# ComputationalRobotics/cuADMM

Hardware: NVIDIA B200
Metric: ADMM iterations/s (higher is better)
Workload: dtype f64

## Files before the change

### cuadmm_b200/csrc/chol_host.cpp

```cpp
#include "chol_host.h"
#include "common.h"
#include <algorithm>
#include <cmath>
#include <numeric>
#include <stdlib.h>

namespace cuadmm {

SymCsc form_aat(int64_t m, int64_t ncols, const int32_t* rowptr, const int32_t* colind, const double* val, double eps) {
    const int64_t nnz = rowptr[m];
    std::vector<int64_t> cp(ncols + 1, 0);
    for (int64_t p = 0; p < nnz; ++p) cp[colind[p] + 1]++;
    for (int64_t k = 0; k < ncols; ++k) cp[k + 1] += cp[k];
    std::vector<int32_t> ci(nnz);
    std::vector<double> cx(nnz);
    {
        std::vector<int64_t> nx(cp.begin(), cp.end() - 1);
        for (int64_t i = 0; i < m; ++i)
            for (int p = rowptr[i]; p < rowptr[i + 1]; ++p) {
                const int64_t q = nx[colind[p]]++;
                ci[q] = (int32_t)i;
                cx[q] = val[p];
            }
    }
    SymCsc M;
    M.n = m;
    M.p.assign(m + 1, 0);
    std::vector<double> acc(m, 0.0);
    std::vector<int32_t> mark(m, -1);
    std::vector<int32_t> list;
    for (int64_t i = 0; i < m; ++i) {
        list.clear();
        mark[i] = (int32_t)i;
        list.push_back((int32_t)i);
        acc[i] = eps;
        for (int p = rowptr[i]; p < rowptr[i + 1]; ++p) {
            const int64_t k = colind[p];
            const double aik = val[p];
            const int32_t* lo = std::lower_bound(ci.data() + cp[k], ci.data() + cp[k + 1], (int32_t)i);
            for (int64_t q = lo - ci.data(); q < cp[k + 1]; ++q) {
                const int32_t j = ci[q];
                if (mark[j] != (int32_t)i) { mark[j] = (int32_t)i; acc[j] = 0.0; list.push_back(j); }
                acc[j] += aik * cx[q];
            }
        }
        std::sort(list.begin(), list.end());
        for (int32_t j : list) { M.i.push_back(j); M.x.push_back(acc[j]); }
        M.p[i + 1] = (int64_t)M.i.size();
    }
    return M;
}

std::vector<int32_t> min_degree_order(const SymCsc& M) {
    const int64_t n = M.n;
    std::vector<int32_t> perm(n);
    if (n == 0) return perm;
    std::vector<std::vector<int32_t>> vadj(n), eadj(n), members(n);
    {
        std::vector<int32_t> cnt(n, 0);
        for (int64_t j = 0; j < n; ++j)
            for (int64_t p = M.p[j]; p < M.p[j + 1]; ++p) if (M.i[p] != j) { cnt[j]++; cnt[M.i[p]]++; }
        for (int64_t j = 0; j < n; ++j) vadj[j].reserve(cnt[j]);
        for (int64_t j = 0; j < n; ++j)
            for (int64_t p = M.p[j]; p < M.p[j + 1]; ++p) if (M.i[p] != j) { vadj[j].push_back(M.i[p]); vadj[M.i[p]].push_back((int32_t)j); }
    }
    enum { VAR = 0, ELEM = 1, DEAD = 2 };
    std::vector<uint8_t> status(n, VAR);
    std::vector<int64_t> degree(n);
    std::vector<int32_t> head(n + 1, -1), next(n, -1), prev(n, -1);
    auto list_insert = [&](int32_t i) {
        const int64_t d = degree[i];
        next[i] = head[d]; prev[i] = -1;
        if (head[d] >= 0) prev[head[d]] = i;
        head[d] = i;
    };
    auto list_remove = [&](int32_t i) {
        const int64_t d = degree[i];
        if (prev[i] >= 0) next[prev[i]] = next[i]; else head[d] = next[i];
        if (next[i] >= 0) prev[next[i]] = prev[i];
    };
    for (int64_t i = 0; i < n; ++i) { degree[i] = (int64_t)vadj[i].size(); }
    for (int64_t i = n - 1; i >= 0; --i) list_insert((int32_t)i);
    std::vector<int64_t> mark(n, -1), wstamp(n, -1), w(n, 0);
    std::vector<int32_t> Lp;
    int64_t mindeg = 0;
    std::vector<int64_t> blocked(n, -1);
    std::vector<int32_t> cands;
    int64_t k = 0, round = 0;
    auto eliminate = [&](const int32_t p) {
        list_remove(p);
        perm[k] = p;
        Lp.clear();
        mark[p] = k;
        for (int32_t v : vadj[p]) if (status[v] == VAR && mark[v] != k) { mark[v] = k; Lp.push_back(v); }
        for (int32_t e : eadj[p]) if (status[e] == ELEM) {
            for (int32_t v : members[e]) if (status[v] == VAR && mark[v] != k) { mark[v] = k; Lp.push_back(v); }
            status[e] = DEAD;
            std::vector<int32_t>().swap(members[e]);
        }
        status[p] = ELEM;
        std::vector<int32_t>().swap(vadj[p]);
        std::vector<int32_t>().swap(eadj[p]);
        const int64_t lp = (int64_t)Lp.size();
        for (int32_t i : Lp) {
            list_remove(i);
            auto& E = eadj[i];
            size_t o = 0;
            for (size_t t = 0; t < E.size(); ++t) {
                const int32_t e = E[t];
                if (status[e] != ELEM) continue;
                if (wstamp[e] != k) { wstamp[e] = k; w[e] = (int64_t)members[e].size(); }
                w[e] -= 1;
                E[o++] = e;
            }
            E.resize(o);
        }
        for (int32_t i : Lp) {
            auto& A = vadj[i];
            size_t o = 0;
            for (size_t t = 0; t < A.size(); ++t) {
                const int32_t v = A[t];
                if (status[v] == VAR && mark[v] != k) A[o++] = v;
            }
            A.resize(o);
            int64_t d = (int64_t)o + (lp - 1);
            auto& E = eadj[i];
            size_t oe = 0;
            for (size_t t = 0; t < E.size(); ++t) {
                const int32_t e = E[t];
                if (status[e] != ELEM) continue;
                if (w[e] <= 0) {
                    status[e] = DEAD;
                    std::vector<int32_t>().swap(members[e]);
                    continue;
                }
                d += w[e];
                E[oe++] = e;
            }
            E.resize(oe);
            E.push_back(p);
            d = std::min<int64_t>(d, n - k - 1);
            d = std::min<int64_t>(d, degree[i] + lp - 1);
            if (d < 0) d = 0;
            degree[i] = d;
        }
        members[p] = Lp;
        for (int32_t i : Lp) {
            list_insert(i);
            blocked[i] = round;
            if (degree[i] < mindeg) mindeg = degree[i];
        }
        ++k;
    };
    const char* slack_env = getenv("CUADMM_MD_SLACK");
    const int64_t slack_pct = slack_env ? atoll(slack_env) : 25;
    while (k < n) {
        ++round;
        while (head[mindeg] < 0) ++mindeg;
        const int64_t limit = std::min<int64_t>(n, mindeg + std::max<int64_t>(1, mindeg * slack_pct / 100));
        cands.clear();
        for (int64_t d = mindeg; d <= limit; ++d)
            for (int32_t i = head[d]; i >= 0; i = next[i]) cands.push_back(i);
        for (int32_t p : cands) {
            if (status[p] != VAR || blocked[p] == round || degree[p] > limit) continue;
            eliminate(p);
        }
    }
    return perm;
}

static SymCsc permute_lower(const SymCsc& M, const std::vector<int32_t>& perm, std::vector<int32_t>& iperm) {
    const int64_t n = M.n;
    iperm.assign(n, 0);
    for (int64_t k = 0; k < n; ++k) iperm[perm[k]] = (int32_t)k;
    SymCsc C;
    C.n = n;
    C.p.assign(n + 1, 0);
    const int64_t nnz = M.p[n];
    for (int64_t j = 0; j < n; ++j)
        for (int64_t p = M.p[j]; p < M.p[j + 1]; ++p) {
            const int32_t a = iperm[j], b = iperm[M.i[p]];
            C.p[std::min(a, b) + 1]++;
        }
    for (int64_t j = 0; j < n; ++j) C.p[j + 1] += C.p[j];
    C.i.resize(nnz); C.x.resize(nnz);
    std::vector<int64_t> nx(C.p.begin(), C.p.end() - 1);
    for (int64_t j = 0; j < n; ++j)
        for (int64_t p = M.p[j]; p < M.p[j + 1]; ++p) {
            const int32_t a = iperm[j], b = iperm[M.i[p]];
            const int64_t q = nx[std::min(a, b)]++;
            C.i[q] = std::max(a, b);
            C.x[q] = M.x[p];
        }
    std::vector<std::pair<int32_t, double>> tmp;
    for (int64_t j = 0; j < n; ++j) {
        tmp.clear();
        for (int64_t p = C.p[j]; p < C.p[j + 1]; ++p) tmp.emplace_back(C.i[p], C.x[p]);
        std::sort(tmp.begin(), tmp.end(), [](const std::pair<int32_t, double>& a, const std::pair<int32_t, double>& b) { return a.first < b.first; });
        for (size_t t = 0; t < tmp.size(); ++t) { C.i[C.p[j] + t] = tmp[t].first; C.x[C.p[j] + t] = tmp[t].second; }
    }
    return C;
}

static void lower_rows(const SymCsc& C, std::vector<int64_t>& rp, std::vector<int32_t>& rj, std::vector<double>& rx) {
    const int64_t n = C.n;
    rp.assign(n + 1, 0);
    for (int64_t j = 0; j < n; ++j)
        for (int64_t p = C.p[j]; p < C.p[j + 1]; ++p) rp[C.i[p] + 1]++;
    for (int64_t i = 0; i < n; ++i) rp[i + 1] += rp[i];
    rj.resize(rp[n]); rx.resize(rp[n]);
    std::vector<int64_t> nx(rp.begin(), rp.end() - 1);
    for (int64_t j = 0; j < n; ++j)
        for (int64_t p = C.p[j]; p < C.p[j + 1]; ++p) {
            const int64_t q = nx[C.i[p]]++;
            rj[q] = (int32_t)j;
            rx[q] = C.x[p];
        }
}

void chol_symbolic(const SymCsc& M, const std::vector<int32_t>& perm, CholFactor& F, SymCsc* permuted) {
    const int64_t n = M.n;
    F.n = n;
    F.perm = perm;
    SymCsc C = permute_lower(M, perm, F.iperm);
    std::vector<int64_t> rp; std::vector<int32_t> rj; std::vector<double> rx;
    lower_rows(C, rp, rj, rx);
    F.parent.assign(n, -1);
    std::vector<int32_t> ancestor(n, -1);
    for (int64_t k = 0; k < n; ++k) {
        for (int64_t p = rp[k]; p < rp[k + 1]; ++p) {
            int32_t i = rj[p];
            while (i != -1 && i < k) {
                const int32_t inext = ancestor[i];
                ancestor[i] = (int32_t)k;
                if (inext == -1) F.parent[i] = (int32_t)k;
                i = inext;
            }
        }
    }
    std::vector<int64_t> cnt(n, 1);
    std::vector<int32_t> flag(n, -1);
    for (int pass = 0; pass < 2; ++pass) {
        std::vector<int64_t> nx;
        if (pass == 1) {
            F.Lp.assign(n + 1, 0);
            for (int64_t j = 0; j < n; ++j) F.Lp[j + 1] = F.Lp[j] + cnt[j];
            F.Li.assign(F.Lp[n], 0);
            F.Lx.assign(F.Lp[n], 0.0);
            nx.assign(F.Lp.begin(), F.Lp.end() - 1);
            for (int64_t j = 0; j < n; ++j) F.Li[nx[j]++] = (int32_t)j;
            std::fill(flag.begin(), flag.end(), -1);
        }
        for (int64_t k = 0; k < n; ++k) {
            flag[k] = (int32_t)k;
            for (int64_t p = rp[k]; p < rp[k + 1]; ++p) {
                int32_t i = rj[p];
                while (i != -1 && i < k && flag[i] != (int32_t)k) {
                    flag[i] = (int32_t)k;
                    if (pass == 0) cnt[i]++; else F.Li[nx[i]++] = (int32_t)k;
                    i = F.parent[i];
                }
            }
        }
    }
    if (permuted) *permuted = std::move(C);
}

std::vector<int32_t> postorder_perm(const SymCsc& M, const std::vector<int32_t>& perm) {
    CholFactor F;
    chol_symbolic(M, perm, F, nullptr);
    const int64_t n = F.n;
    std::vector<int32_t> head(n, -1), nxt(n, -1);
    for (int64_t j = n - 1; j >= 0; --j) if (F.parent[j] >= 0) { nxt[j] = head[F.parent[j]]; head[F.parent[j]] = (int32_t)j; }
    std::vector<int32_t> post; post.reserve(n);
    std::vector<int32_t> stack;
    for (int64_t r = 0; r < n; ++r) {
        if (F.parent[r] >= 0) continue;
        stack.push_back((int32_t)r);
        while (!stack.empty()) {
            const int32_t v = stack.back();
            const int32_t c = head[v];
            if (c >= 0) { head[v] = nxt[c]; stack.push_back(c); }
            else { post.push_back(v); stack.pop_back(); }
        }
    }
    std::vector<int32_t> out(n);
    for (int64_t k = 0; k < n; ++k) out[k] = perm[post[k]];
    return out;
}

std::vector<int64_t> find_supernodes(const CholFactor& F, int64_t max_size) {
    const int64_t n = F.n;
    std::vector<int64_t> sn;
    sn.push_back(0);
    std::vector<int32_t> nchild(n, 0);
    for (int64_t j = 0; j < n; ++j) if (F.parent[j] >= 0) nchild[F.parent[j]]++;
    for (int64_t j = 1; j < n; ++j) {
        const int64_t cprev = F.Lp[j] - F.Lp[j - 1], ccur = F.Lp[j + 1] - F.Lp[j];
        const bool join = F.parent[j - 1] == j && ccur == cprev - 1 && nchild[j] == 1 && (j - sn.back()) < max_size;
        if (!join) sn.push_back(j);
    }
    if (n > 0) sn.push_back(n);
    return sn;
}

double pivot_tol() {
    if (const char* e = getenv("CUADMM_PIVOT_TOL")) { const double v = atof(e); if (v > 0.0 && v < 1.0) return v; }
    return 1e-11;
}

void chol_numeric(const SymCsc& C, CholFactor& F, int64_t n_lead) {
    F.n_deficient = 0;
    const double kPivotTol = pivot_tol();
    const int64_t n = F.n;
    std::vector<int64_t> rp; std::vector<int32_t> rj; std::vector<double> rx;
    lower_rows(C, rp, rj, rx);
    std::vector<double> x(n, 0.0);
    std::vector<int64_t> c(n);
    for (int64_t j = 0; j < n; ++j) c[j] = F.Lp[j] + 1;
    std::vector<int32_t> flag(n, -1), stack(n), path(n);
    for (int64_t k = 0; k < n; ++k) {
        int64_t top = n;
        flag[k] = (int32_t)k;
        double d = 0.0, mkk = 0.0;
        for (int64_t p = rp[k]; p < rp[k + 1]; ++p) {
            int32_t i = rj[p];
            if (i == k) { d = rx[p]; mkk = rx[p]; continue; }
            x[i] = rx[p];
            int64_t len = 0;
            while (i != -1 && i < k && flag[i] != (int32_t)k) {
                path[len++] = i;
                flag[i] = (int32_t)k;
                i = F.parent[i];
            }
            while (len > 0) stack[--top] = path[--len];
        }
        for (; top < n; ++top) {
            const int32_t i = stack[top];
            if (i >= n_lead) { x[i] = 0.0; continue; }
            const double lki = x[i] / F.Lx[F.Lp[i]];
            x[i] = 0.0;
            const int64_t pend = c[i];
            if (k < n_lead) {
                for (int64_t p = F.Lp[i] + 1; p < pend; ++p) x[F.Li[p]] -= F.Lx[p] * lki;
            } else {
                for (int64_t p = F.Lp[i] + 1; p < pend && F.Li[p] < n_lead; ++p) x[F.Li[p]] -= F.Lx[p] * lki;
            }
            d -= lki * lki;
            F.Lx[pend] = lki;
            c[i] = pend + 1;
        }
        if (k < n_lead) {
            if (!(d > kPivotTol * std::max(mkk, 1e-300))) {
                F.Lx[F.Lp[k]] = INFINITY;
                F.n_deficient++;
            } else {
                F.Lx[F.Lp[k]] = std::sqrt(d);
            }
        } else {
            F.Lx[F.Lp[k]] = d;
        }
    }
}

}
```

### cuadmm_b200/csrc/chol_host.h

```cpp
#pragma once
#include <stdint.h>
#include <vector>

namespace cuadmm {

struct SymCsc {
    int64_t n = 0;
    std::vector<int64_t> p;
    std::vector<int32_t> i;
    std::vector<double> x;
};

SymCsc form_aat(int64_t m, int64_t ncols, const int32_t* rowptr, const int32_t* colind, const double* val, double eps);

std::vector<int32_t> min_degree_order(const SymCsc& M);

struct CholFactor {
    int64_t n = 0;
    std::vector<int32_t> perm, iperm;
    std::vector<int32_t> parent;
    std::vector<int64_t> Lp;
    std::vector<int32_t> Li;
    std::vector<double> Lx;
    int64_t n_deficient = 0;
    int64_t nnz() const { return Lp.empty() ? 0 : Lp[n]; }
};

std::vector<int32_t> postorder_perm(const SymCsc& M, const std::vector<int32_t>& perm);

std::vector<int64_t> find_supernodes(const CholFactor& F, int64_t max_size);

void chol_symbolic(const SymCsc& M, const std::vector<int32_t>& perm, CholFactor& F, SymCsc* permuted = nullptr);
double pivot_tol();
void chol_numeric(const SymCsc& Mperm, CholFactor& F, int64_t n_lead);

}
```

### cuadmm_b200/csrc/debug_api.cpp

```cpp
#include "chol_host.h"
#include "common.h"
#include <algorithm>
#include <cmath>

using namespace cuadmm;

extern "C" {

int cuadmm_debug_chol_solve(int64_t m, int64_t ncols, const int32_t* rowptr, const int32_t* colind, const double* val,
                            double eps, double n_lead_frac, const double* rhs, double* y, int32_t* perm_out,
                            int64_t* stats ) {
    return guarded([&] {
        SymCsc M = form_aat(m, ncols, rowptr, colind, val, eps);
        std::vector<int32_t> perm = min_degree_order(M);
        perm = postorder_perm(M, perm);
        CholFactor F; SymCsc C;
        chol_symbolic(M, perm, F, &C);
        const int64_t n_lead = std::max<int64_t>(0, std::min<int64_t>(m, (int64_t)(n_lead_frac * (double)m)));
        chol_numeric(C, F, n_lead);
        const int64_t r = m - n_lead;
        std::vector<double> S((size_t)(r * r), 0.0);
        for (int64_t j = n_lead; j < m; ++j)
            for (int64_t p = C.p[j]; p < C.p[j + 1]; ++p) S[(C.i[p] - n_lead) + (j - n_lead) * r] = C.x[p];
        for (int64_t j = 0; j < n_lead; ++j)
            for (int64_t p = F.Lp[j] + 1; p < F.Lp[j + 1]; ++p) if (F.Li[p] >= n_lead)
                for (int64_t q = p; q < F.Lp[j + 1]; ++q)
                    S[(F.Li[q] - n_lead) + (F.Li[p] - n_lead) * r] -= F.Lx[q] * F.Lx[p];
        for (int64_t k = 0; k < r; ++k) {
            double d = S[k + k * r];
            d = (d > 1e-11) ? std::sqrt(d) : INFINITY; S[k + k * r] = d;
            for (int64_t i = k + 1; i < r; ++i) S[i + k * r] /= d;
            for (int64_t j = k + 1; j < r; ++j)
                for (int64_t i = j; i < r; ++i) S[i + j * r] -= S[i + k * r] * S[j + k * r];
        }
        std::vector<double> z(m);
        for (int64_t k = 0; k < m; ++k) z[k] = rhs[F.perm[k]];
        for (int64_t j = 0; j < n_lead; ++j) {
            z[j] /= F.Lx[F.Lp[j]];
            for (int64_t p = F.Lp[j] + 1; p < F.Lp[j + 1]; ++p) z[F.Li[p]] -= F.Lx[p] * z[j];
        }
        for (int64_t j = 0; j < r; ++j) {
            z[n_lead + j] /= S[j + j * r];
            for (int64_t i = j + 1; i < r; ++i) z[n_lead + i] -= S[i + j * r] * z[n_lead + j];
        }
        for (int64_t j = r - 1; j >= 0; --j) {
            for (int64_t i = j + 1; i < r; ++i) z[n_lead + j] -= S[i + j * r] * z[n_lead + i];
            z[n_lead + j] /= S[j + j * r];
        }
        for (int64_t j = n_lead - 1; j >= 0; --j) {
            for (int64_t p = F.Lp[j] + 1; p < F.Lp[j + 1]; ++p) z[j] -= F.Lx[p] * z[F.Li[p]];
            z[j] /= F.Lx[F.Lp[j]];
        }
        for (int64_t k = 0; k < m; ++k) y[F.perm[k]] = z[k];
        if (perm_out) std::copy(F.perm.begin(), F.perm.end(), perm_out);
        if (stats) {
            stats[0] = M.p[m]; stats[1] = F.nnz(); stats[2] = F.n_deficient;
            std::vector<int32_t> lev(m, 0);
            int32_t depth = 0;
            for (int64_t j = 0; j < m; ++j) {
                for (int64_t p = F.Lp[j] + 1; p < F.Lp[j + 1]; ++p) lev[F.Li[p]] = std::max(lev[F.Li[p]], lev[j] + 1);
                depth = std::max(depth, lev[j] + 1);
            }
            stats[3] = depth;
            std::vector<int64_t> cnt(depth + 1, 0);
            for (int64_t j = 0; j < m; ++j) cnt[lev[j]]++;
            int64_t narrow = 0;
            for (int32_t l = 0; l < depth; ++l) if (cnt[l] < 8) narrow += cnt[l];
            stats[4] = narrow;
            std::vector<int64_t> sn = find_supernodes(F, 256);
            const int64_t nsn = (int64_t)sn.size() - 1;
            std::vector<int32_t> snof(m, 0), slev(std::max<int64_t>(nsn, 1), 0);
            for (int64_t s = 0; s < nsn; ++s) for (int64_t j = sn[s]; j < sn[s + 1]; ++j) snof[j] = (int32_t)s;
            int32_t sdepth = 0;
            for (int64_t s = 0; s < nsn; ++s) {
                for (int64_t j = sn[s]; j < sn[s + 1]; ++j)
                    for (int64_t p = F.Lp[j] + 1; p < F.Lp[j + 1]; ++p) {
                        const int32_t t = snof[F.Li[p]];
                        if (t != s) slev[t] = std::max(slev[t], slev[s] + 1);
                    }
                sdepth = std::max(sdepth, slev[s] + 1);
            }
            stats[5] = nsn; stats[6] = sdepth;
            std::vector<int64_t> scnt(sdepth + 1, 0);
            for (int64_t s = 0; s < nsn; ++s) scnt[slev[s]] += sn[s + 1] - sn[s];
            int64_t deep_rows = 0;
            for (int32_t l = 48; l < sdepth; ++l) deep_rows += scnt[l];
            stats[7] = deep_rows;
        }
    });
}

}
```

### cuadmm_b200/csrc/dense.cu

```cuda
#include "dense.h"
#include <stdio.h>
#include <stdlib.h>
#include <algorithm>

namespace cuadmm {

static constexpr int GB_M = 64, GB_N = 64, GB_K = 16, GB_PAD = 4;

__device__ __forceinline__ void dmma_m8n8k4(double& c0, double& c1, double a, double b) {
    asm volatile("mma.sync.aligned.m8n8k4.row.col.f64.f64.f64.f64 {%0,%1}, {%2}, {%3}, {%0,%1};"
                 : "+d"(c0), "+d"(c1) : "d"(a), "d"(b));
}

template <bool TA, bool TB>
__global__ void __launch_bounds__(128) dgemm_kernel(int64_t m, int64_t n, int64_t k, double alpha,
                                                    const double* __restrict__ A, int64_t lda,
                                                    const double* __restrict__ B, int64_t ldb,
                                                    double beta, double* C, int64_t ldc, int shape) {
    if (shape == 1 && (int64_t)blockIdx.y * GB_N > (int64_t)blockIdx.x * GB_M + (GB_M - 1)) return;
    __shared__ double As[2][GB_K][GB_M + GB_PAD];
    __shared__ double Bs[2][GB_K][GB_N + GB_PAD];
    const int tid = threadIdx.x, lane = tid & 31, warp = tid >> 5;
    const int wm = (warp & 1) * 32, wn = (warp >> 1) * 32;
    const int64_t m0 = (int64_t)blockIdx.x * GB_M, n0 = (int64_t)blockIdx.y * GB_N;
    double acc[4][4][2];
#pragma unroll
    for (int i = 0; i < 4; ++i)
#pragma unroll
        for (int j = 0; j < 4; ++j) { acc[i][j][0] = 0.0; acc[i][j][1] = 0.0; }

    auto load_tiles = [&](int buf, int64_t k0) {
#pragma unroll
        for (int t = 0; t < 8; ++t) {
            const int e = tid + t * 128;
            int mm, kk;
            if (TA) { kk = e % GB_K; mm = e / GB_K; } else { mm = e % GB_M; kk = e / GB_M; }
            const int64_t gm = m0 + mm, gk = k0 + kk;
            double v = 0.0;
            if (gm < m && gk < k) v = TA ? A[gk + gm * lda] : A[gm + gk * lda];
            As[buf][kk][mm] = v;
        }
#pragma unroll
        for (int t = 0; t < 8; ++t) {
            const int e = tid + t * 128;
            int nn, kk;
            if (TB) { nn = e % GB_N; kk = e / GB_N; } else { kk = e % GB_K; nn = e / GB_K; }
            const int64_t gn = n0 + nn, gk = k0 + kk;
            double v = 0.0;
            if (gn < n && gk < k) v = TB ? B[gn + gk * ldb] : B[gk + gn * ldb];
            Bs[buf][kk][nn] = v;
        }
    };

    const int64_t nk = (k + GB_K - 1) / GB_K;
    const int64_t kt0 = (shape == 2) ? ((n0 / GB_K < nk) ? n0 / GB_K : nk) : 0;
    if (nk > kt0) load_tiles((int)(kt0 & 1), kt0 * GB_K);
    __syncthreads();
    for (int64_t kt = kt0; kt < nk; ++kt) {
        const int buf = (int)(kt & 1);
        if (kt + 1 < nk) load_tiles(buf ^ 1, (kt + 1) * GB_K);
#pragma unroll
        for (int kk = 0; kk < GB_K; kk += 4) {
            double a[4], b[4];
#pragma unroll
            for (int i = 0; i < 4; ++i) a[i] = As[buf][kk + (lane & 3)][wm + i * 8 + (lane >> 2)];
#pragma unroll
            for (int j = 0; j < 4; ++j) b[j] = Bs[buf][kk + (lane & 3)][wn + j * 8 + (lane >> 2)];
#pragma unroll
            for (int i = 0; i < 4; ++i)
#pragma unroll
                for (int j = 0; j < 4; ++j) dmma_m8n8k4(acc[i][j][0], acc[i][j][1], a[i], b[j]);
        }
        __syncthreads();
    }
#pragma unroll
    for (int i = 0; i < 4; ++i)
#pragma unroll
        for (int j = 0; j < 4; ++j)
#pragma unroll
            for (int h = 0; h < 2; ++h) {
                const int64_t gm = m0 + wm + i * 8 + (lane >> 2);
                const int64_t gn = n0 + wn + j * 8 + (lane & 3) * 2 + h;
                if (gm < m && gn < n) {
                    double* c = C + gm + gn * ldc;
                    *c = (beta == 0.0) ? alpha * acc[i][j][h] : alpha * acc[i][j][h] + beta * (*c);
                }
            }
}

void dgemm(cudaStream_t st, bool transA, bool transB, int64_t m, int64_t n, int64_t k, double alpha,
           const double* A, int64_t lda, const double* B, int64_t ldb, double beta, double* C, int64_t ldc, int shape) {
    if (m <= 0 || n <= 0) return;
    dim3 grid((unsigned)((m + GB_M - 1) / GB_M), (unsigned)((n + GB_N - 1) / GB_N));
    if (!transA && !transB) dgemm_kernel<false, false><<<grid, 128, 0, st>>>(m, n, k, alpha, A, lda, B, ldb, beta, C, ldc, shape);
    else if (!transA && transB) dgemm_kernel<false, true><<<grid, 128, 0, st>>>(m, n, k, alpha, A, lda, B, ldb, beta, C, ldc, shape);
    else if (transA && !transB) dgemm_kernel<true, false><<<grid, 128, 0, st>>>(m, n, k, alpha, A, lda, B, ldb, beta, C, ldc, shape);
    else dgemm_kernel<true, true><<<grid, 128, 0, st>>>(m, n, k, alpha, A, lda, B, ldb, beta, C, ldc, shape);
    CUADMM_CUDA(cudaGetLastError());
}

static constexpr int NB = 64;

__global__ void __launch_bounds__(256) potf2_inv_kernel(int nb, double* A, int64_t lda, double* inv, int* info, int blk_index, const double* pivot_floor) {
    extern __shared__ double potf2_smem[];
    double (*S)[NB + 1] = reinterpret_cast<double (*)[NB + 1]>(potf2_smem);
    double (*I)[NB + 1] = reinterpret_cast<double (*)[NB + 1]>(potf2_smem + NB * (NB + 1));
    __shared__ int bad;
    const int tid = threadIdx.x;
    if (tid == 0) bad = 0;
    for (int e = tid; e < nb * nb; e += 256) { const int i = e % nb, j = e / nb; S[i][j] = (i >= j) ? A[i + j * lda] : 0.0; }
    __syncthreads();
    for (int kk = 0; kk < nb; ++kk) {
        if (tid == 0) {
            const double d = S[kk][kk];
            const double fl = pivot_floor ? pivot_floor[kk] : 0.0;
            if (!(d > fl)) { bad = 1; S[kk][kk] = INFINITY; } else S[kk][kk] = sqrt(d);
        }
        __syncthreads();
        const double dk = S[kk][kk];
        for (int i = kk + 1 + tid; i < nb; i += 256) S[i][kk] /= dk;
        __syncthreads();
        const int rem = nb - kk - 1;
        for (int e = tid; e < rem * rem; e += 256) {
            const int i = kk + 1 + e % rem, j = kk + 1 + e / rem;
            if (i >= j) S[i][j] -= S[i][kk] * S[j][kk];
        }
        __syncthreads();
    }
    if (tid < nb) {
        const int j = tid;
        for (int i = 0; i < nb; ++i) {
            double s = (i == j) ? 1.0 : 0.0;
            for (int t = j; t < i; ++t) s -= S[i][t] * I[t][j];
            I[i][j] = (i >= j) ? s / S[i][i] : 0.0;
        }
    }
    __syncthreads();
    for (int e = tid; e < nb * nb; e += 256) {
        const int i = e % nb, j = e / nb;
        if (i >= j) A[i + j * lda] = S[i][j];
        if (inv) inv[i + (int64_t)j * NB] = I[i][j];
    }
    if (tid == 0 && bad && info) atomicAdd(info, 1);
}

void potrf_lower(cudaStream_t st, int64_t n, double* A, int64_t lda, double* inv_diag, int* d_info, const double* pivot_floor) {
    DevBuf<double> tmp(std::max<int64_t>(n * NB, 1));
    DevBuf<double> inv_local;
    if (!inv_diag) { inv_local.alloc(std::max<int64_t>(n * NB, 1)); inv_diag = inv_local.p; }
    const size_t potf2_bytes = sizeof(double) * 2 * NB * (NB + 1);
    CUADMM_CUDA(cudaFuncSetAttribute((const void*)potf2_inv_kernel, cudaFuncAttributeMaxDynamicSharedMemorySize, (int)potf2_bytes));
    for (int64_t j = 0; j < n; j += NB) {
        const int nb = (int)std::min<int64_t>(NB, n - j);
        double* Ajj = A + j + j * lda;
        double* invj = inv_diag + j * NB;
        potf2_inv_kernel<<<1, 256, potf2_bytes, st>>>(nb, Ajj, lda, invj, d_info, (int)(j / NB), pivot_floor ? pivot_floor + j : nullptr);
        const int64_t below = n - j - nb;
        if (below > 0) {
            double* Aij = A + (j + nb) + j * lda;
            dgemm(st, false, true, below, nb, nb, 1.0, Aij, lda, invj, NB, 0.0, tmp.p, below);
            CUADMM_CUDA(cudaMemcpy2DAsync(Aij, sizeof(double) * lda, tmp.p, sizeof(double) * below,
                                          sizeof(double) * below, nb, cudaMemcpyDeviceToDevice, st));
            double* A22 = A + (j + nb) + (j + nb) * lda;
            dgemm(st, false, true, below, below, nb, -1.0, Aij, lda, Aij, lda, 1.0, A22, lda, 1);
        }
    }
    CUADMM_CUDA(cudaGetLastError());
    CUADMM_CUDA(cudaStreamSynchronize(st));
}

__global__ void copy_inv_block_kernel(int nb, const double* __restrict__ inv, double* X, int64_t ldx) {
    for (int e = threadIdx.x; e < nb * nb; e += blockDim.x) {
        const int i = e % nb, j = e / nb;
        X[i + j * ldx] = inv[i + (int64_t)j * NB];
    }
}

void trtri_lower(cudaStream_t st, int64_t n, const double* L, int64_t ldl, const double* inv_diag, double* X, int64_t ldx) {
    CUADMM_CUDA(cudaMemset2DAsync(X, sizeof(double) * ldx, 0, sizeof(double) * n, n, st));
    DevBuf<double> T(std::max<int64_t>((int64_t)NB * n, 1));
    for (int64_t i = 0; i < n; i += NB) {
        const int nb = (int)std::min<int64_t>(NB, n - i);
        const double* invi = inv_diag + i * NB;
        copy_inv_block_kernel<<<1, 256, 0, st>>>(nb, invi, X + i + i * ldx, ldx);
        if (i > 0) {
            dgemm(st, false, false, nb, i, i, 1.0, L + i, ldl, X, ldx, 0.0, T.p, NB, 2);
            dgemm(st, false, false, nb, i, nb, -1.0, invi, NB, T.p, NB, 0.0, X + i, ldx);
        }
    }
    CUADMM_CUDA(cudaGetLastError());
    CUADMM_CUDA(cudaStreamSynchronize(st));
}

__global__ void scatter_coo_kernel(int64_t nnz, const int32_t* __restrict__ r, const int32_t* __restrict__ c,
                                   const double* __restrict__ v, double* D, int64_t ld, int symmetric) {
    const int64_t e = (int64_t)blockIdx.x * blockDim.x + threadIdx.x;
    if (e >= nnz) return;
    D[r[e] + (int64_t)c[e] * ld] = v[e];
    if (symmetric && r[e] != c[e]) D[c[e] + (int64_t)r[e] * ld] = v[e];
}

__global__ void transpose_kernel(int64_t n, const double* __restrict__ in, double* __restrict__ out) {
    __shared__ double tile[32][33];
    const int64_t bx = (int64_t)blockIdx.x * 32, by = (int64_t)blockIdx.y * 32;
    for (int j = threadIdx.y; j < 32; j += blockDim.y) {
        const int64_t x = bx + threadIdx.x, y = by + j;
        if (x < n && y < n) tile[j][threadIdx.x] = in[x + y * n];
    }
    __syncthreads();
    for (int j = threadIdx.y; j < 32; j += blockDim.y) {
        const int64_t x = by + threadIdx.x, y = bx + j;
        if (x < n && y < n) out[x + y * n] = tile[threadIdx.x][j];
    }
}

__global__ void tile_occupancy_kernel(int64_t r, int nt, const double* __restrict__ A, int* __restrict__ flags) {
    const int I = blockIdx.y, J = blockIdx.x;
    int any = 0;
    for (int e = threadIdx.x; e < 64 * 64; e += blockDim.x) {
        const int64_t i = (int64_t)I * 64 + e / 64, j = (int64_t)J * 64 + e % 64;
        if (i < r && j < r && A[i * r + j] != 0.0) any = 1;
    }
    if (__syncthreads_or(any) && threadIdx.x == 0) flags[I * nt + J] = 1;
}

void build_dense_tail(const SymCsc& C, const CholFactor& F, int64_t n_lead, int64_t r,
                      DevBuf<double>& tail_inv, DevBuf<double>& tail_inv_t, int64_t* n_deficient,
                      std::vector<int>* tile_flags) {
    cudaStream_t st = 0;
    DevBuf<double> S(r * r);
    S.zero(st);
    {
        std::vector<int32_t> rr, cc; std::vector<double> vv;
        for (int64_t j = n_lead; j < n_lead + r; ++j)
            for (int64_t p = C.p[j]; p < C.p[j + 1]; ++p) { rr.push_back((int32_t)(C.i[p] - n_lead)); cc.push_back((int32_t)(j - n_lead)); vv.push_back(C.x[p]); }
        if (!vv.empty()) {
            DevBuf<int32_t> dr, dc; DevBuf<double> dv;
            dr.upload(rr, st); dc.upload(cc, st); dv.upload(vv, st);
            scatter_coo_kernel<<<(unsigned)((vv.size() + 255) / 256), 256, 0, st>>>((int64_t)vv.size(), dr.p, dc.p, dv.p, S.p, r, 1);
            CUADMM_CUDA(cudaStreamSynchronize(st));
        }
    }
    {
        std::vector<int64_t> cols;
        for (int64_t j = 0; j < n_lead; ++j)
            if (F.Lp[j + 1] > F.Lp[j] + 1 && F.Li[F.Lp[j + 1] - 1] >= n_lead) cols.push_back(j);
        const int64_t budget = (int64_t)1 << 27;
        const int64_t cw = std::max<int64_t>(64, std::min<int64_t>((int64_t)cols.size(), budget / std::max<int64_t>(r, 1)));
        DevBuf<double> B(r * std::min<int64_t>(cw, std::max<int64_t>((int64_t)cols.size(), 1)));
        std::vector<int32_t> rr, cc; std::vector<double> vv;
        for (int64_t c0 = 0; c0 < (int64_t)cols.size(); c0 += cw) {
            const int64_t w = std::min<int64_t>(cw, (int64_t)cols.size() - c0);
            rr.clear(); cc.clear(); vv.clear();
            for (int64_t t = 0; t < w; ++t) {
                const int64_t j = cols[c0 + t];
                for (int64_t p = F.Lp[j + 1] - 1; p > F.Lp[j] && F.Li[p] >= n_lead; --p) {
                    rr.push_back((int32_t)(F.Li[p] - n_lead)); cc.push_back((int32_t)t); vv.push_back(F.Lx[p]);
                }
            }
            CUADMM_CUDA(cudaMemsetAsync(B.p, 0, sizeof(double) * (size_t)(r * w), st));
            DevBuf<int32_t> dr, dc; DevBuf<double> dv;
            dr.upload(rr, st); dc.upload(cc, st); dv.upload(vv, st);
            scatter_coo_kernel<<<(unsigned)((vv.size() + 255) / 256), 256, 0, st>>>((int64_t)vv.size(), dr.p, dc.p, dv.p, B.p, r, 0);
            dgemm(st, false, true, r, r, w, -1.0, B.p, r, B.p, r, 1.0, S.p, r, 1);
            CUADMM_CUDA(cudaStreamSynchronize(st));
        }
    }
    DevBuf<double> inv_diag(std::max<int64_t>(r * NB, 1));
    DevBuf<int> info(1);
    info.zero(st);
    std::vector<double> h_floor(r, 0.0);
    for (int64_t j = n_lead; j < n_lead + r; ++j)
        for (int64_t p = C.p[j]; p < C.p[j + 1]; ++p) if (C.i[p] == j) h_floor[j - n_lead] = pivot_tol() * C.x[p];
    DevBuf<double> d_floor; d_floor.upload(h_floor, st);
    potrf_lower(st, r, S.p, r, inv_diag.p, info.p, d_floor.p);
    int h_info = 0;
    info.download(&h_info, 1, st);
    CUADMM_CUDA(cudaStreamSynchronize(st));
    if (n_deficient) *n_deficient = h_info;
    tail_inv_t.alloc(r * r);
    trtri_lower(st, r, S.p, r, inv_diag.p, tail_inv_t.p, r);
    tail_inv.alloc(r * r);
    dim3 grid((unsigned)((r + 31) / 32), (unsigned)((r + 31) / 32)), block(32, 8);
    transpose_kernel<<<grid, block, 0, st>>>(r, tail_inv_t.p, tail_inv.p);
    CUADMM_CUDA(cudaGetLastError());
    CUADMM_CUDA(cudaStreamSynchronize(st));
    {
        const int nt = (int)((r + 63) / 64);
        DevBuf<int> flags((int64_t)nt * nt);
        flags.zero(st);
        tile_occupancy_kernel<<<dim3(nt, nt), 256, 0, st>>>(r, nt, tail_inv.p, flags.p);
        std::vector<int> h((size_t)nt * nt);
        flags.download(h.data(), (int64_t)h.size(), st);
        CUADMM_CUDA(cudaStreamSynchronize(st));
        if (getenv("CUADMM_YSOLVE_VERBOSE")) {
            int64_t lower = 0, used = 0;
            for (int I = 0; I < nt; ++I) for (int J = 0; J <= I; ++J) { ++lower; used += h[(size_t)I * nt + J]; }
            fprintf(stderr, "[ysolve] dense tail %lld: %lld of %lld lower 64x64 tiles of L22^-1 are non-zero (%.1f%%)\n",
                    (long long)r, (long long)used, (long long)lower, 100.0 * (double)used / (double)lower);
        }
        if (tile_flags) tile_flags->swap(h);
    }
}

}
```

### cuadmm_b200/csrc/dense.h

```cpp
#pragma once
#include "common.h"
#include "chol_host.h"

namespace cuadmm {

void dgemm(cudaStream_t st, bool transA, bool transB, int64_t m, int64_t n, int64_t k, double alpha,
           const double* A, int64_t lda, const double* B, int64_t ldb, double beta, double* C, int64_t ldc, int shape = 0);

void potrf_lower(cudaStream_t st, int64_t n, double* A, int64_t lda, double* inv_diag, int* d_info,
                 const double* pivot_floor = nullptr);
void trtri_lower(cudaStream_t st, int64_t n, const double* L, int64_t ldl, const double* inv_diag, double* Linv, int64_t ldi);

void build_dense_tail(const SymCsc& Cperm, const CholFactor& F, int64_t n_lead, int64_t n_tail,
                      DevBuf<double>& tail_inv, DevBuf<double>& tail_inv_t, int64_t* n_deficient = nullptr,
                      std::vector<int>* tile_flags = nullptr);

}
```

### cuadmm_b200/csrc/ysolve.cu

```cuda
#include "ysolve.h"
#include <chrono>
#include <thread>
#include <atomic>
#include "dense.h"
#include <algorithm>
#include <numeric>
#include <stdio.h>
#include <stdlib.h>

namespace cuadmm {

static constexpr int kTriThreads = 256;
static constexpr int kLongRowNnz = 24;
static constexpr int kNarrowSlots = 160;
static constexpr int kNarrowThreads = 1024;

struct SlotWork {
    static constexpr int K = 4;
    int32_t u; int is_long;
    double rv, invd;
    int64_t p, p1; int step;
    int32_t d[K]; double v[K];

    __device__ __forceinline__ void load(int64_t s, int lane, const int32_t* __restrict__ slot_rows,
            const int32_t* __restrict__ slot_info, const int64_t* __restrict__ ptr, const int32_t* __restrict__ dep,
            const double* __restrict__ val, const double* __restrict__ inv_diag, const double* __restrict__ rhs,
            const int32_t* __restrict__ rhs_gather) {
        is_long = slot_info[s] >> 30;
        u = slot_rows[8 * s + (is_long ? 0 : (lane >> 2))];
        step = is_long ? 32 : 4;
        p = 0; p1 = 0; rv = 0.0; invd = 0.0;
        if (u >= 0) {
            p = ptr[u] + (is_long ? lane : (lane & 3));
            p1 = ptr[u + 1];
            invd = inv_diag[u];
            rv = rhs_gather ? rhs[rhs_gather[u]] : rhs[u];
        }
#pragma unroll
        for (int k = 0; k < K; ++k) {
            const int64_t q = p + (int64_t)k * step;
            if (q < p1) { d[k] = dep[q]; v[k] = val[q]; } else { d[k] = -1; v[k] = 0.0; }
        }
    }
    __device__ __forceinline__ void finish(int lane, const int32_t* __restrict__ dep, const double* __restrict__ val,
                                           double* x, double* out_scatter, const int32_t* __restrict__ out_perm) {
        double acc = 0.0;
#pragma unroll
        for (int k = 0; k < K; ++k) if (d[k] >= 0) acc = fma(v[k], x[d[k]], acc);
        for (int64_t q = p + (int64_t)K * step; q < p1; q += step) acc = fma(val[q], x[dep[q]], acc);
        acc += __shfl_xor_sync(0xffffffffu, acc, 1);
        acc += __shfl_xor_sync(0xffffffffu, acc, 2);
        if (is_long) {
            acc += __shfl_xor_sync(0xffffffffu, acc, 4);
            acc += __shfl_xor_sync(0xffffffffu, acc, 8);
            acc += __shfl_xor_sync(0xffffffffu, acc, 16);
        }
        const bool writer = (u >= 0) && (is_long ? (lane == 0) : ((lane & 3) == 0));
        if (writer) {
            const double r = (rv - acc) * invd;
            x[u] = r;
            if (out_scatter) out_scatter[out_perm[u]] = r;
        }
    }
};

#define CUADMM_TRI_PARAMS                                                                                   \
    const int32_t* __restrict__ slot_rows, const int32_t* __restrict__ slot_info, const int64_t* __restrict__ ptr, \
    const int32_t* __restrict__ dep, const double* __restrict__ val, const double* __restrict__ inv_diag,   \
    const double* __restrict__ rhs, const int32_t* __restrict__ rhs_gather, double* x, double* out_scatter, \
    const int32_t* __restrict__ out_perm, const int* __restrict__ done_flag
#define CUADMM_TRI_LOAD(W, S) (W).load((S), lane, slot_rows, slot_info, ptr, dep, val, inv_diag, rhs, rhs_gather)
#define CUADMM_TRI_FINISH(W) (W).finish(lane, dep, val, x, out_scatter, out_perm)

__global__ void __launch_bounds__(kTriThreads) tri_wide_kernel(int64_t slot0, int64_t slot1, CUADMM_TRI_PARAMS) {
    if (done_flag && *done_flag) return;
    const int lane = threadIdx.x & 31;
    const int64_t s = slot0 + (((int64_t)blockIdx.x * kTriThreads + threadIdx.x) >> 5);
    if (s >= slot1) return;
    SlotWork w;
    CUADMM_TRI_LOAD(w, s);
    CUADMM_TRI_FINISH(w);
}

template <int NW>
__device__ __forceinline__ void tri_level_loop(const int64_t* __restrict__ lvl_ptr, int level0, int level1, int lane, int warp,
        CUADMM_TRI_PARAMS) {
    (void)done_flag;
    if (level0 >= level1) return;
    SlotWork w;
    int64_t s0 = lvl_ptr[level0];
    int64_t s1 = lvl_ptr[level0 + 1];
    bool have = (s0 + warp) < s1;
    if (have) CUADMM_TRI_LOAD(w, s0 + warp);
    for (int l = level0; l < level1; ++l) {
        if (have) {
            CUADMM_TRI_FINISH(w);
            for (int64_t s = s0 + warp + NW; s < s1; s += NW) { SlotWork t; CUADMM_TRI_LOAD(t, s); CUADMM_TRI_FINISH(t); }
        }
        s0 = s1;
        have = false;
        if (l + 1 < level1) {
            s1 = lvl_ptr[l + 2];
            have = (s0 + warp) < s1;
            if (have) CUADMM_TRI_LOAD(w, s0 + warp);
        }
        __syncthreads();
    }
}

__global__ void __launch_bounds__(kNarrowThreads) tri_narrow_kernel(int level0, int level1, const int64_t* __restrict__ level_ptr,
                                                                    CUADMM_TRI_PARAMS) {
    if (done_flag && *done_flag) return;
    tri_level_loop<kNarrowThreads / 32>(level_ptr, level0, level1, threadIdx.x & 31, threadIdx.x >> 5,
        slot_rows, slot_info, ptr, dep, val, inv_diag, rhs, rhs_gather, x, out_scatter, out_perm, done_flag);
}

__global__ void __launch_bounds__(kTriThreads) tri_subtree_kernel(const int64_t* __restrict__ sub_off,
        const int64_t* __restrict__ sub_lvl_ptr, CUADMM_TRI_PARAMS) {
    if (done_flag && *done_flag) return;
    const int64_t base = sub_off[blockIdx.x];
    const int nl = (int)(sub_off[blockIdx.x + 1] - base) - 1;
    tri_level_loop<kTriThreads / 32>(sub_lvl_ptr + base, 0, nl, threadIdx.x & 31, threadIdx.x >> 5,
        slot_rows, slot_info, ptr, dep, val, inv_diag, rhs, rhs_gather, x, out_scatter, out_perm, done_flag);
}

#ifndef CUADMM_PK_CHUNK
#define CUADMM_PK_CHUNK 65536
#endif
#ifndef CUADMM_PK_RING
#define CUADMM_PK_RING 2
#endif
static constexpr int kPkChunk = CUADMM_PK_CHUNK;
static constexpr int kPkRing = CUADMM_PK_RING;
#ifndef CUADMM_PK_THREADS
#define CUADMM_PK_THREADS 1024
#endif
static constexpr int kPkThreads = CUADMM_PK_THREADS;
static constexpr int kPkRecHeader = 8 + 32 + 16 + 16 + 16 + 64;
static constexpr int kPkMaxRowEntries = 768;
static constexpr int kPkMaxRows = 23000;
static constexpr int kPkChainMax = 384;

__device__ __forceinline__ uint32_t smem_u32(const void* p) { return (uint32_t)__cvta_generic_to_shared(p); }

__device__ __forceinline__ long long pk_globaltimer() {
    long long t;
    asm volatile("mov.u64 %0, %%globaltimer;" : "=l"(t));
    return t;
}

__device__ __forceinline__ void pk_fetch(unsigned char* dst, const unsigned char* src, uint64_t* bar) {
    asm volatile("mbarrier.arrive.expect_tx.shared::cta.b64 _, [%0], %1;" :: "r"(smem_u32(bar)), "r"(kPkChunk) : "memory");
    asm volatile("cp.async.bulk.shared::cluster.global.mbarrier::complete_tx::bytes [%0], [%1], %2, [%3];"
                 :: "r"(smem_u32(dst)), "l"(src), "r"(kPkChunk), "r"(smem_u32(bar)) : "memory");
}

__device__ __forceinline__ void pk_wait(uint64_t* bar, uint32_t parity) {
    uint32_t ok;
    do {
        asm volatile("{ .reg .pred p; mbarrier.try_wait.parity.shared::cta.b64 p, [%1], %2; selp.u32 %0, 1, 0, p; }"
                     : "=r"(ok) : "r"(smem_u32(bar)), "r"(parity) : "memory");
    } while (!ok);
}

__device__ __forceinline__ void pk_record(const unsigned char* rec, int lane, double* xs) {
    const int r = lane >> 2;
    const bool is_long = *reinterpret_cast<const int32_t*>(rec) != 0;
    const int ul = reinterpret_cast<const int32_t*>(rec + 8)[r];
    const int voff = reinterpret_cast<const uint16_t*>(rec + 40)[r];
    const int ioff = reinterpret_cast<const uint16_t*>(rec + 56)[r];
    const int ln = reinterpret_cast<const uint16_t*>(rec + 72)[r];
    const double invd = reinterpret_cast<const double*>(rec + 88)[r];
    const int j = is_long ? lane : (lane & 3);
    const int step = is_long ? 32 : 4;
    const double* val = reinterpret_cast<const double*>(rec) + voff;
    const uint16_t* idx = reinterpret_cast<const uint16_t*>(rec) + ioff;
    const double cur = ul >= 0 ? xs[ul] : 0.0;
    double acc = 0.0;
    for (int k = j; k < ln; k += step) acc = fma(val[k], xs[idx[k]], acc);
    acc += __shfl_xor_sync(0xffffffffu, acc, 1);
    acc += __shfl_xor_sync(0xffffffffu, acc, 2);
    if (is_long) {
        acc += __shfl_xor_sync(0xffffffffu, acc, 4);
        acc += __shfl_xor_sync(0xffffffffu, acc, 8);
        acc += __shfl_xor_sync(0xffffffffu, acc, 16);
    }
    if (ul >= 0 && j == 0) xs[ul] = (cur - acc) * invd;
}

static constexpr int kPkHeavyExt = 8;

__global__ void __launch_bounds__(256) pk_gather_kernel(int64_t n_rows, int main_blocks, const int32_t* __restrict__ heavy,
        int n_heavy, const int32_t* __restrict__ prow_src, const int64_t* __restrict__ ext_ptr,
        const int32_t* __restrict__ ext_dep, const double* __restrict__ ext_val, const double* __restrict__ rhs,
        const double* __restrict__ x, double* __restrict__ w, const int* __restrict__ done_flag) {
    if (done_flag && *done_flag) return;
    if ((int)blockIdx.x < main_blocks) {
        const int64_t g = (int64_t)blockIdx.x * 256 + threadIdx.x;
        if (g >= n_rows) return;
        const int32_t src = prow_src[g];
        double acc = src >= 0 ? rhs[src] : 0.0;
        if (ext_ptr) {
            const int64_t p0 = ext_ptr[g], p1 = ext_ptr[g + 1];
            if (p1 - p0 > kPkHeavyExt) return;
            for (int64_t p = p0; p < p1; ++p) acc = fma(-ext_val[p], x[ext_dep[p]], acc);
        }
        w[g] = acc;
    } else {
        const int lane = threadIdx.x & 31;
        const int hw = ((int)blockIdx.x - main_blocks) * 8 + (threadIdx.x >> 5);
        if (hw >= n_heavy) return;
        const int64_t g = heavy[hw];
        double acc = 0.0;
        for (int64_t p = ext_ptr[g] + lane; p < ext_ptr[g + 1]; p += 32) acc = fma(ext_val[p], x[ext_dep[p]], acc);
#pragma unroll
        for (int o = 16; o > 0; o >>= 1) acc += __shfl_xor_sync(0xffffffffu, acc, o);
        if (lane == 0) {
            const int32_t src = prow_src[g];
            w[g] = (src >= 0 ? rhs[src] : 0.0) - acc;
        }
    }
}

__device__ __forceinline__ void pk_record2(const unsigned char* recA, const unsigned char* recB, bool hasB, int lane, double* xs) {
    const int r = lane >> 2;
    const bool longA = *reinterpret_cast<const int32_t*>(recA) != 0;
    const bool longB = *reinterpret_cast<const int32_t*>(recB) != 0;
    const int ulA = reinterpret_cast<const int32_t*>(recA + 8)[r];
    const int ulB = hasB ? reinterpret_cast<const int32_t*>(recB + 8)[r] : -1;
    const int voffA = reinterpret_cast<const uint16_t*>(recA + 40)[r], voffB = reinterpret_cast<const uint16_t*>(recB + 40)[r];
    const int ioffA = reinterpret_cast<const uint16_t*>(recA + 56)[r], ioffB = reinterpret_cast<const uint16_t*>(recB + 56)[r];
    const int lnA = reinterpret_cast<const uint16_t*>(recA + 72)[r];
    const int lnB = hasB ? reinterpret_cast<const uint16_t*>(recB + 72)[r] : 0;
    const double invdA = reinterpret_cast<const double*>(recA + 88)[r], invdB = reinterpret_cast<const double*>(recB + 88)[r];
    const int jA = longA ? lane : (lane & 3), jB = longB ? lane : (lane & 3);
    const int stepA = longA ? 32 : 4, stepB = longB ? 32 : 4;
    const double* valA = reinterpret_cast<const double*>(recA) + voffA;
    const double* valB = reinterpret_cast<const double*>(recB) + voffB;
    const uint16_t* idxA = reinterpret_cast<const uint16_t*>(recA) + ioffA;
    const uint16_t* idxB = reinterpret_cast<const uint16_t*>(recB) + ioffB;
    const double curA = ulA >= 0 ? xs[ulA] : 0.0;
    const double curB = ulB >= 0 ? xs[ulB] : 0.0;
    double accA = 0.0, accB = 0.0;
    int kA = jA, kB = jB;
    while (kA < lnA || kB < lnB) {
        const bool a = kA < lnA, b = kB < lnB;
        double va = 0.0, vb = 0.0;
        int ia = 0, ib = 0;
        if (a) { va = valA[kA]; ia = idxA[kA]; }
        if (b) { vb = valB[kB]; ib = idxB[kB]; }
        const double xa = xs[ia], xb = xs[ib];
        if (a) accA = fma(va, xa, accA);
        if (b) accB = fma(vb, xb, accB);
        kA += stepA; kB += stepB;
    }
    accA += __shfl_xor_sync(0xffffffffu, accA, 1);
    accB += __shfl_xor_sync(0xffffffffu, accB, 1);
    accA += __shfl_xor_sync(0xffffffffu, accA, 2);
    accB += __shfl_xor_sync(0xffffffffu, accB, 2);
    if (longA || longB) {
        double tA = accA, tB = accB;
        tA += __shfl_xor_sync(0xffffffffu, tA, 4);  tB += __shfl_xor_sync(0xffffffffu, tB, 4);
        tA += __shfl_xor_sync(0xffffffffu, tA, 8);  tB += __shfl_xor_sync(0xffffffffu, tB, 8);
        tA += __shfl_xor_sync(0xffffffffu, tA, 16); tB += __shfl_xor_sync(0xffffffffu, tB, 16);
        if (longA) accA = tA;
        if (longB) accB = tB;
    }
    if (ulA >= 0 && jA == 0) xs[ulA] = (curA - accA) * invdA;
    if (ulB >= 0 && jB == 0) xs[ulB] = (curB - accB) * invdB;
}

template <int NW, bool WARP>
__device__ __forceinline__ void pk_chunk(const unsigned char* chunk, int lane, int warp, double* xs) {
    const uint16_t* dir = reinterpret_cast<const uint16_t*>(chunk);
    const int nseg = dir[0];
    const uint16_t* seg_end = dir + 2;
    const uint16_t* rec_off = seg_end + nseg;
    int sb = 0;
    for (int g = 0; g < nseg; ++g) {
        const int se = seg_end[g];
        int sl = sb + warp;
        if constexpr (!WARP) {
            for (; sl + NW < se; sl += 2 * NW)
                pk_record2(chunk + 8 * (int)rec_off[sl], chunk + 8 * (int)rec_off[sl + NW], true, lane, xs);
        }
        for (; sl < se; sl += NW) pk_record(chunk + 8 * (int)rec_off[sl], lane, xs);
        if constexpr (WARP) __syncwarp(); else __syncthreads();
        sb = se;
    }
}

__global__ void __launch_bounds__(kPkThreads, 1) tri_packed_kernel(const int64_t* __restrict__ chunk_off,
        const int64_t* __restrict__ row_off, const unsigned char* __restrict__ stream, const int32_t* __restrict__ prow_u,
        const int32_t* __restrict__ prow_out, const double* __restrict__ w, double* x, double* out_scatter,
        const int* __restrict__ done_flag, long long* __restrict__ timeline) {
    if (done_flag && *done_flag) return;
    if (timeline && threadIdx.x == 0) timeline[4 * blockIdx.x + 0] = pk_globaltimer();
    extern __shared__ __align__(128) unsigned char pk_smem[];
    unsigned char* ring = pk_smem;
    uint64_t* bars = reinterpret_cast<uint64_t*>(pk_smem + kPkRing * kPkChunk);
    double* xs = reinterpret_cast<double*>(pk_smem + kPkRing * kPkChunk + 64);
    const int tid = threadIdx.x, lane = tid & 31, warp = tid >> 5;
    const int64_t c0 = chunk_off[blockIdx.x];
    const int nc = (int)(chunk_off[blockIdx.x + 1] - c0);
    const int64_t r0 = row_off[blockIdx.x];
    const int nr = (int)(row_off[blockIdx.x + 1] - r0);
    const unsigned char* src = stream + c0 * kPkChunk;
    if (tid == 0) {
        for (int i = 0; i < kPkRing; ++i)
            asm volatile("mbarrier.init.shared::cta.b64 [%0], 1;" :: "r"(smem_u32(bars + i)) : "memory");
        asm volatile("fence.mbarrier_init.release.cluster;" ::: "memory");
        asm volatile("fence.proxy.async.shared::cta;" ::: "memory");
        for (int i = 0; i < kPkRing && i < nc; ++i) pk_fetch(ring + i * kPkChunk, src + (int64_t)i * kPkChunk, bars + i);
    }
#pragma unroll 4
    for (int loc = tid; loc < nr; loc += kPkThreads) xs[loc] = w[r0 + loc];
    __syncthreads();
    if (timeline && tid == 0) timeline[4 * blockIdx.x + 1] = pk_globaltimer();
    for (int c = 0; c < nc; ++c) {
        const int b = c % kPkRing;
        pk_wait(bars + b, (uint32_t)((c / kPkRing) & 1));
        pk_chunk<kPkThreads / 32, false>(ring + b * kPkChunk, lane, warp, xs);
        if (tid == 0 && c + kPkRing < nc) pk_fetch(ring + b * kPkChunk, src + (int64_t)(c + kPkRing) * kPkChunk, bars + b);
    }
    if (timeline && tid == 0) timeline[4 * blockIdx.x + 2] = pk_globaltimer();
#pragma unroll 4
    for (int loc = tid; loc < nr; loc += kPkThreads) {
        const int32_t u = prow_u[r0 + loc];
        if (u < 0) continue;
        const double r = xs[loc];
        x[u] = r;
        if (out_scatter) out_scatter[prow_out[r0 + loc]] = r;
    }
    if (timeline && tid == 0) timeline[4 * blockIdx.x + 3] = pk_globaltimer();
}

static constexpr int kPkWarpBlob = 2048;
static constexpr int kPkWarpRows = 32;
static constexpr int kPkWarpThreads = 256;

__global__ void __launch_bounds__(kPkWarpThreads, 5) tri_packed_warp_kernel(int64_t count, const int64_t* __restrict__ blob_off,
        const int64_t* __restrict__ row_off, const uint4* __restrict__ blobs, const int32_t* __restrict__ prow_u,
        const int32_t* __restrict__ prow_out, const double* __restrict__ w, double* x, double* out_scatter,
        const int* __restrict__ done_flag) {
    if (done_flag && *done_flag) return;
    __shared__ __align__(16) unsigned char slices[kPkWarpThreads / 32][kPkWarpBlob];
    __shared__ double xs_all[kPkWarpThreads / 32][kPkWarpRows];
    const int lane = threadIdx.x & 31, warp = threadIdx.x >> 5;
    const int64_t t = (int64_t)blockIdx.x * (kPkWarpThreads / 32) + warp;
    if (t >= count) return;
    const int64_t b0 = blob_off[t];
    const int nb = (int)(blob_off[t + 1] - b0);
    const int64_t r0 = row_off[t];
    const int nr = (int)(row_off[t + 1] - r0);
    uint4* slice = reinterpret_cast<uint4*>(slices[warp]);
    double* xs = xs_all[warp];
    for (int i = lane; i < nb; i += 32) slice[i] = blobs[b0 + i];
    int32_t u = -1, po = -1;
    if (lane < nr) {
        xs[lane] = w[r0 + lane];
        u = prow_u[r0 + lane];
        if (out_scatter) po = prow_out[r0 + lane];
    }
    __syncwarp();
    pk_chunk<1, true>(slices[warp], lane, 0, xs);
    if (lane < nr && u >= 0) {
        const double r = xs[lane];
        x[u] = r;
        if (out_scatter) out_scatter[po] = r;
    }
}

__global__ void __launch_bounds__(256) tail_gemv_row_kernel(int64_t r, const double* __restrict__ T, const double* __restrict__ in,
                                                        double* out, const int32_t* __restrict__ tile_ptr,
                                                        const int32_t* __restrict__ tile_col, double* out_scatter,
                                                        const int32_t* __restrict__ out_perm, int64_t perm_base,
                                                        const int* __restrict__ done_flag, int longest_last) {
    if (done_flag && *done_flag) return;
    const int lane = threadIdx.x & 31;
    const int64_t cta = longest_last ? (int64_t)gridDim.x - 1 - blockIdx.x : blockIdx.x;
    const int64_t row = cta * (blockDim.x >> 5) + (threadIdx.x >> 5);
    if (row >= r) return;
    const double* Ti = T + row * r;
    const int I = (int)(row >> 6);
    double acc0 = 0.0, acc1 = 0.0;
    const bool vec = (r & 1) == 0 && (reinterpret_cast<uintptr_t>(T) & 15) == 0;
    const bool in_al = (reinterpret_cast<uintptr_t>(in) & 15) == 0;
    for (int t = tile_ptr[I]; t < tile_ptr[I + 1]; ++t) {
        const int64_t j0 = tile_col[2 * t];
        const int64_t j1 = min((int64_t)tile_col[2 * t + 1], r);
        if (vec) {
            const int64_t jv = j0 + ((j1 - j0) & ~(int64_t)1);
#pragma unroll 4
            for (int64_t j = j0 + 2 * lane; j < jv; j += 64) {
                const double2 a = __ldcs(reinterpret_cast<const double2*>(Ti + j));
                const double2 b = in_al ? *reinterpret_cast<const double2*>(in + j) : make_double2(in[j], in[j + 1]);
                acc0 = fma(a.x, b.x, acc0);
                acc1 = fma(a.y, b.y, acc1);
            }
            if (lane == 0 && jv < j1) acc0 = fma(Ti[jv], in[jv], acc0);
        } else {
#pragma unroll 4
            for (int64_t j = j0 + lane; j < j1; j += 32) acc0 = fma(Ti[j], in[j], acc0);
        }
    }
    double acc = acc0 + acc1;
#pragma unroll
    for (int o = 16; o > 0; o >>= 1) acc += __shfl_xor_sync(0xffffffffu, acc, o);
    if (lane == 0) {
        out[row] = acc;
        if (out_scatter) out_scatter[out_perm[perm_base + row]] = acc;
    }
}

__global__ void __launch_bounds__(256) tail_gemv_kernel(int64_t r, const double* __restrict__ T, const double* in,
                                                        double* out, const int32_t* __restrict__ tile_ptr,
                                                        const int32_t* __restrict__ tile_col, double* out_scatter,
                                                        const int32_t* __restrict__ out_perm, int64_t perm_base,
                                                        const int* __restrict__ done_flag, int longest_last,
                                                        int64_t row0, int64_t nrows, int npush, PeerView pv,
                                                        PeerPtrs outp, PeerPtrs scatp, int splits, double* split_part,
                                                        unsigned int* split_count) {
    if (done_flag && *done_flag) return;
    __shared__ double part[8][9];
    __shared__ int s_final;
    const int lane = threadIdx.x & 31, w = threadIdx.x >> 5;
    unsigned long long ep = 0;
    if (npush) ep = peer_epoch(pv);
    const int sp = (int)(blockIdx.x % (unsigned)splits);
    const int64_t rb = blockIdx.x / (unsigned)splits, nrb = gridDim.x / (unsigned)splits;
    const int64_t cta = longest_last ? nrb - 1 - rb : rb;
    const int64_t base = row0 + cta * 8;
    const int nr = (int)max((int64_t)0, min((int64_t)8, row0 + nrows - base));
    double acc[8];
#pragma unroll
    for (int q = 0; q < 8; ++q) acc[q] = 0.0;
    if (nr > 0) {
        const int I = (int)(base >> 6);
        const bool vec = (r & 1) == 0 && (reinterpret_cast<uintptr_t>(T) & 15) == 0 && (reinterpret_cast<uintptr_t>(in) & 15) == 0;
        const double* Tb = T + base * r;
        int g = 0;
        for (int t = tile_ptr[I]; t < tile_ptr[I + 1]; ++t) {
            const int64_t j0 = tile_col[2 * t];
            const int64_t j1 = min((int64_t)tile_col[2 * t + 1], r);
            const int nch = (int)((j1 - j0 + 63) >> 6);
            const int g0 = g;
            int c = (w - (g & 7)) & 7;
            g += nch;
            for (; c < nch; c += 8) {
                if (splits > 1 && (((g0 + c) >> 3) % splits) != sp) continue;
                const int64_t j = j0 + ((int64_t)c << 6) + 2 * lane;
                if (vec) {
                    if (j + 1 < j1) {
                        const double2 b = *reinterpret_cast<const double2*>(in + j);
#pragma unroll
                        for (int q = 0; q < 8; ++q) {
                            if (q < nr) {
                                const double2 a = __ldcs(reinterpret_cast<const double2*>(Tb + q * r + j));
                                acc[q] = fma(a.x, b.x, fma(a.y, b.y, acc[q]));
                            }
                        }
                    } else if (j < j1) {
                        const double b = in[j];
#pragma unroll
                        for (int q = 0; q < 8; ++q) if (q < nr) acc[q] = fma(Tb[q * r + j], b, acc[q]);
                    }
                } else {
#pragma unroll
                    for (int h = 0; h < 2; ++h) {
                        const int64_t jj = j0 + ((int64_t)c << 6) + lane + 32 * h;
                        if (jj < j1) {
                            const double b = in[jj];
#pragma unroll
                            for (int q = 0; q < 8; ++q) if (q < nr) acc[q] = fma(Tb[q * r + jj], b, acc[q]);
                        }
                    }
                }
            }
        }
    }
#pragma unroll
    for (int q = 0; q < 8; ++q) {
#pragma unroll
        for (int o = 16; o > 0; o >>= 1) acc[q] += __shfl_xor_sync(0xffffffffu, acc[q], o);
    }
    if (lane == 0) {
#pragma unroll
        for (int q = 0; q < 8; ++q) part[w][q] = acc[q];
    }
    __syncthreads();
    const int t = threadIdx.x;
    bool final_cta = true;
    if (splits > 1) {
        if (t < 8) {
            double v = 0.0;
#pragma unroll
            for (int k = 0; k < 8; ++k) v += part[k][t];
            split_part[(rb * splits + sp) * 8 + t] = v;
        }
        __syncthreads();
        if (t == 0) {
            __threadfence();
            const unsigned old = atomicAdd(split_count + rb, 1u);
            s_final = (old == (unsigned)splits - 1u) ? 1 : 0;
            if (s_final) { split_count[rb] = 0u; __threadfence(); }
        }
        __syncthreads();
        final_cta = s_final != 0;
    }
    if (final_cta && t < 8 * max(npush, 1)) {
        const int q = t >> 3, rr = t & 7;
        if (rr < nr) {
            double v = 0.0;
            if (splits > 1) {
                for (int k = 0; k < splits; ++k) v += __ldcg(split_part + (rb * splits + k) * 8 + rr);
            } else {
#pragma unroll
                for (int k = 0; k < 8; ++k) v += part[k][rr];
            }
            if (npush == 0) {
                out[base + rr] = v;
                if (out_scatter) out_scatter[out_perm[perm_base + base + rr]] = v;
            } else {
                outp.p[q][base + rr] = v;
            }
        }
    }
    if (npush) peer_leave(pv, ep);
}

__global__ void __launch_bounds__(256) tail_scatter_kernel(int64_t r, const double* __restrict__ xt, const int32_t* __restrict__ perm,
                                                           int64_t base, double* y, const int* __restrict__ done_flag) {
    if (done_flag && *done_flag) return;
    const int64_t i = (int64_t)blockIdx.x * 256 + threadIdx.x;
    if (i < r) y[perm[base + i]] = xt[i];
}

static int launch_subtrees(const TriSweep& S, const double* rhs, const int32_t* gather, double* x, double* out_scatter,
                           const int32_t* out_perm, const int* done, cudaStream_t st, const SweepStreams& ss) {
    int launches = 0;
    if (S.pk_rows > 0) {
        const int main_blocks = (int)((S.pk_rows + 255) / 256);
        pk_gather_kernel<<<(unsigned)(main_blocks + (S.pk_n_heavy + 7) / 8), 256, 0, st>>>(S.pk_rows, main_blocks, S.pk_heavy.p,
            (int)S.pk_n_heavy, S.pk_prow_src.p, S.pk_has_ext ? S.pk_ext_ptr.p : nullptr, S.pk_ext_dep.p, S.pk_ext_val.p, rhs, x,
            S.pk_w.p, done);
        ++launches;
    }
    const bool fork = S.n_sub_warp > 0 && (S.n_sub_pack > 0 || S.n_sub_cta > 0);
    cudaStream_t wst = st;
    if (fork) {
        CUADMM_CUDA(cudaEventRecord(ss.fork, st));
        CUADMM_CUDA(cudaStreamWaitEvent(ss.side, ss.fork, 0));
        wst = ss.side;
    }
    if (S.n_sub_pack > 0) {
        tri_packed_kernel<<<(unsigned)S.n_sub_pack, kPkThreads, S.pk_smem, st>>>(S.pk_chunk_off.p, S.pk_row_off.p, S.pk_stream.p,
            S.pk_prow_u.p, S.pk_prow_out.p, S.pk_w.p, x, out_scatter, done, S.pk_timeline.n ? S.pk_timeline.p : nullptr);
        ++launches;
    }
    if (S.n_sub_warp > 0) {
        const int wpb = kPkWarpThreads / 32;
        tri_packed_warp_kernel<<<(unsigned)((S.n_sub_warp + wpb - 1) / wpb), kPkWarpThreads, 0, wst>>>(S.n_sub_warp,
            S.pk_blob_off.p, S.pk_row_off.p + S.n_sub_pack, reinterpret_cast<const uint4*>(S.pk_blobs.p), S.pk_prow_u.p,
            S.pk_prow_out.p, S.pk_w.p, x, out_scatter, done);
        ++launches;
    }
    if (S.n_sub_cta > 0) {
        tri_subtree_kernel<<<(unsigned)S.n_sub_cta, kTriThreads, 0, st>>>(S.sub_off.p, S.sub_lvl_ptr.p, S.slot_rows.p, S.slot_info.p,
            S.ptr.p, S.dep.p, S.val.p, S.inv_diag.p, rhs, gather, x, out_scatter, out_perm, done);
        ++launches;
    }
    if (fork) {
        CUADMM_CUDA(cudaEventRecord(ss.join, ss.side));
        CUADMM_CUDA(cudaStreamWaitEvent(st, ss.join, 0));
    }
    return launches;
}

static int launch_sweep(const TriSweep& S, const double* rhs, const int32_t* gather, double* x,
                        double* out_scatter, const int32_t* out_perm, const int* done, cudaStream_t st, const SweepStreams& ss) {
    int launches = 0;
    if (S.subtrees_first && S.n_sub) launches += launch_subtrees(S, rhs, gather, x, out_scatter, out_perm, done, st, ss);
    for (const TriSweep::Phase& ph : S.phases) {
        if (ph.narrow) {
            tri_narrow_kernel<<<1, kNarrowThreads, 0, st>>>(ph.level0, ph.level1, S.level_ptr.p, S.slot_rows.p, S.slot_info.p,
                S.ptr.p, S.dep.p, S.val.p, S.inv_diag.p, rhs, gather, x, out_scatter, out_perm, done);
        } else {
            const int64_t s0 = S.h_level_ptr[ph.level0], s1 = S.h_level_ptr[ph.level1];
            const int grid = (int)(((s1 - s0) * 32 + kTriThreads - 1) / kTriThreads);
            tri_wide_kernel<<<grid, kTriThreads, 0, st>>>(s0, s1, S.slot_rows.p, S.slot_info.p, S.ptr.p, S.dep.p, S.val.p,
                S.inv_diag.p, rhs, gather, x, out_scatter, out_perm, done);
        }
        ++launches;
    }
    if (!S.subtrees_first && S.n_sub) launches += launch_subtrees(S, rhs, gather, x, out_scatter, out_perm, done, st, ss);
    CUADMM_CUDA(cudaGetLastError());
    return launches;
}

struct HostSweep {
    std::vector<int64_t> ptr;
    std::vector<int32_t> dep;
    std::vector<double> val, inv_diag;
    int64_t n = 0;
    std::vector<int32_t> order;
    std::vector<int32_t> sub;
    int64_t n_sub = 0;
    bool subtrees_first = true;
    const std::vector<int32_t>* gather = nullptr;
    const std::vector<int32_t>* out_perm = nullptr;
};

static int64_t emit_level_slots(const HostSweep& H, std::vector<int32_t>& rows, int level,
                                std::vector<int32_t>& slot_rows, std::vector<int32_t>& slot_info) {
    std::vector<int32_t> longs, shorts;
    for (int32_t u : rows) ((H.ptr[u + 1] - H.ptr[u]) > kLongRowNnz ? longs : shorts).push_back(u);
    std::stable_sort(longs.begin(), longs.end(), [&](int32_t a, int32_t b) {
        return H.ptr[a + 1] - H.ptr[a] > H.ptr[b + 1] - H.ptr[b]; });
    int64_t cnt = 0;
    for (int32_t u : longs) {
        slot_rows.push_back(u);
        for (int t = 1; t < 8; ++t) slot_rows.push_back(-1);
        slot_info.push_back(level | (1 << 30));
        ++cnt;
    }
    for (size_t t = 0; t < shorts.size(); t += 8) {
        for (size_t q = t; q < t + 8; ++q) slot_rows.push_back(q < shorts.size() ? shorts[q] : -1);
        slot_info.push_back(level);
        ++cnt;
    }
    return cnt;
}

struct PkRow {
    int32_t slot; double invd;
    std::vector<uint16_t> idx; std::vector<double> val;
};

static void pack_subtrees(const HostSweep& H, TriSweep& S, const std::vector<std::vector<int32_t>>& members,
                          const std::vector<int32_t>& level, const std::vector<int32_t>& depth, std::vector<int>& kind) {
    struct Packed {
        std::vector<unsigned char> bytes; int32_t t; size_t last_used; int levels;
        std::vector<int32_t> slot_u, slot_src;
    };
    std::vector<Packed> packs, blobs;
    std::vector<int32_t> loc(H.n, -1), cidx(H.n, -1), height(H.n, 0), lvl_r(H.n, 0);
    int chain_max = kPkChainMax, chain_gain = 6;
    if (const char* e = getenv("CUADMM_SWEEP_CHAIN_MAX")) chain_max = std::min(atoi(e), kPkMaxRowEntries);
    const bool verbose = getenv("CUADMM_YSOLVE_VERBOSE") != nullptr;
    int64_t n_collapsed = 0, levels_before = 0, levels_after = 0, chain_entries = 0;
    kind.assign(H.n_sub, 0);
    auto same = [&](int32_t u, int64_t p) { return H.sub[H.dep[p]] == H.sub[u]; };
    std::vector<Packed> result(H.n_sub);
    std::atomic<int64_t> a_collapsed{0}, a_before{0}, a_after{0}, a_entries{0};
    auto do_subtree = [&](int64_t t) {
        const std::vector<int32_t>& rows = members[t];
        const int32_t nr0 = (int32_t)rows.size();
        if (nr0 + chain_max > kPkMaxRows) return;
        int32_t longest = 0;
        for (int32_t q = 0; q < nr0; ++q) {
            const int32_t u = rows[q];
            loc[u] = q;
            int32_t cnt = 0;
            for (int64_t p = H.ptr[u]; p < H.ptr[u + 1]; ++p) cnt += same(u, p) ? 1 : 0;
            longest = std::max(longest, cnt);
        }
        if (longest > kPkMaxRowEntries) return;
        std::vector<int32_t> C;
        int new_depth = depth[t], k0 = 0;
        if (chain_max > 0 && depth[t] > chain_gain + 2 && nr0 > kPkWarpRows) {
            const bool initial = !H.subtrees_first;
            std::vector<int32_t> key(nr0);
            if (initial) {
                for (int32_t u : rows) height[u] = 0;
                for (int32_t q = nr0 - 1; q >= 0; --q) {
                    const int32_t u = rows[q];
                    for (int64_t p = H.ptr[u]; p < H.ptr[u + 1]; ++p)
                        if (same(u, p)) height[H.dep[p]] = std::max(height[H.dep[p]], height[u] + 1);
                }
                for (int32_t q = 0; q < nr0; ++q) key[q] = height[rows[q]];
            } else {
                for (int32_t q = 0; q < nr0; ++q) key[q] = level[rows[q]];
            }
            std::vector<int32_t> cnt(depth[t] + 1, 0);
            for (int32_t q = 0; q < nr0; ++q) ++cnt[key[q]];
            int32_t acc = 0;
            k0 = depth[t];
            while (k0 > 0 && acc + cnt[k0 - 1] <= chain_max) { --k0; acc += cnt[k0]; }
            const int nd = initial ? k0 + 1 : k0 + 2;
            if (acc > 0 && depth[t] - nd >= chain_gain) {
                new_depth = nd;
                for (int32_t q = 0; q < nr0; ++q) if (key[q] >= k0) C.push_back(rows[q]);
            }
        }
        const int32_t nC = (int32_t)C.size();
        for (int32_t i = 0; i < nC; ++i) cidx[C[i]] = i;
        std::vector<std::vector<PkRow>> lv(new_depth);
        auto plain_row = [&](int32_t u) {
            PkRow r; r.slot = loc[u]; r.invd = H.inv_diag[u];
            for (int64_t p = H.ptr[u]; p < H.ptr[u + 1]; ++p)
                if (same(u, p)) { r.idx.push_back((uint16_t)loc[H.dep[p]]); r.val.push_back(H.val[p]); }
            return r;
        };
        if (nC == 0) {
            for (int32_t u : rows) lv[level[u]].push_back(plain_row(u));
        } else {
            std::vector<double> M((size_t)nC * nC, 0.0);
            for (int32_t i = 0; i < nC; ++i) {
                const int32_t u = C[i];
                double* mi = M.data() + (size_t)i * nC;
                mi[i] = 1.0;
                for (int64_t p = H.ptr[u]; p < H.ptr[u + 1]; ++p) {
                    if (!same(u, p) || cidx[H.dep[p]] < 0) continue;
                    const int32_t k = cidx[H.dep[p]];
                    const double v = H.val[p];
                    const double* mk = M.data() + (size_t)k * nC;
                    for (int32_t j = 0; j <= k; ++j) mi[j] -= v * mk[j];
                }
                const double d = H.inv_diag[u];
                for (int32_t j = 0; j <= i; ++j) mi[j] *= d;
            }
            const bool initial = !H.subtrees_first;
            const int lvB = initial ? 0 : k0 + 1;
            for (int32_t i = 0; i < nC; ++i) {
                PkRow r; r.slot = loc[C[i]]; r.invd = -1.0;
                const double* mi = M.data() + (size_t)i * nC;
                for (int32_t j = 0; j <= i; ++j) if (mi[j] != 0.0) { r.idx.push_back((uint16_t)(nr0 + j)); r.val.push_back(mi[j]); }
                a_entries += (int64_t)r.idx.size();
                lv[lvB].push_back(std::move(r));
            }
            if (initial) {
                for (int32_t u : rows) {
                    if (cidx[u] >= 0) continue;
                    int32_t l = 0;
                    for (int64_t p = H.ptr[u]; p < H.ptr[u + 1]; ++p)
                        if (same(u, p) && cidx[H.dep[p]] < 0) l = std::max(l, lvl_r[H.dep[p]] + 1);
                    lvl_r[u] = l;
                    lv[1 + l].push_back(plain_row(u));
                }
            } else {
                for (int32_t u : rows) {
                    if (cidx[u] < 0) { lv[level[u]].push_back(plain_row(u)); continue; }
                    PkRow r; r.slot = nr0 + cidx[u]; r.invd = 1.0;
                    for (int64_t p = H.ptr[u]; p < H.ptr[u + 1]; ++p)
                        if (same(u, p) && cidx[H.dep[p]] < 0) { r.idx.push_back((uint16_t)loc[H.dep[p]]); r.val.push_back(H.val[p]); }
                    if (!r.idx.empty()) lv[k0].push_back(std::move(r));
                }
            }
            ++a_collapsed; a_before += depth[t]; a_after += new_depth;
        }
        Packed& P = result[t]; P.t = (int32_t)t; P.last_used = 0; P.levels = new_depth;
        P.slot_u.assign(nr0 + nC, -1); P.slot_src.assign(nr0 + nC, -1);
        for (int32_t q = 0; q < nr0; ++q) {
            const int32_t u = rows[q];
            P.slot_u[q] = u;
            if (cidx[u] < 0) P.slot_src[q] = u; else P.slot_src[nr0 + cidx[u]] = u;
        }
        std::vector<uint16_t> seg_end, rec_rel;
        std::vector<unsigned char> recs;
        auto dir_bytes = [](size_t nseg, size_t nslots) { return (4 + 2 * nseg + 2 * nslots + 7) / 8 * 8; };
        auto close_chunk = [&]() {
            if (rec_rel.empty()) return;
            seg_end.push_back((uint16_t)rec_rel.size());
            const size_t db = dir_bytes(seg_end.size(), rec_rel.size());
            if (!P.bytes.empty()) P.bytes.resize((P.bytes.size() + kPkChunk - 1) / kPkChunk * kPkChunk, 0);
            std::vector<unsigned char> chunk((db + recs.size() + 15) / 16 * 16, 0);
            uint16_t* dir = reinterpret_cast<uint16_t*>(chunk.data());
            dir[0] = (uint16_t)seg_end.size(); dir[1] = (uint16_t)rec_rel.size();
            for (size_t i = 0; i < seg_end.size(); ++i) dir[2 + i] = seg_end[i];
            for (size_t i = 0; i < rec_rel.size(); ++i) dir[2 + seg_end.size() + i] = (uint16_t)((db + rec_rel[i]) / 8);
            CUADMM_REQUIRE(db + recs.size() <= (size_t)kPkChunk, "internal: packed chunk overflow");
            std::copy(recs.begin(), recs.end(), chunk.begin() + db);
            P.bytes.insert(P.bytes.end(), chunk.begin(), chunk.end());
            P.last_used = db + recs.size();
            seg_end.clear(); rec_rel.clear(); recs.clear();
        };
        auto add_record = [&](const std::vector<unsigned char>& rec, bool new_level) {
            const size_t nseg = seg_end.size() + 1 + ((new_level && !rec_rel.empty()) ? 1 : 0);
            if (dir_bytes(nseg, rec_rel.size() + 1) + recs.size() + rec.size() > (size_t)kPkChunk) close_chunk();
            if (new_level && !rec_rel.empty()) seg_end.push_back((uint16_t)rec_rel.size());
            rec_rel.push_back((uint16_t)recs.size());
            recs.insert(recs.end(), rec.begin(), rec.end());
        };
        auto make_record = [&](const PkRow* const* rs, int nrows, bool is_long) {
            size_t ne = 0;
            for (int r = 0; r < nrows; ++r) ne += rs[r]->val.size();
            const size_t val0 = kPkRecHeader, idx0 = kPkRecHeader + 8 * ne;
            std::vector<unsigned char> rec(idx0 + (2 * ne + 7) / 8 * 8, 0);
            int32_t* hdr = reinterpret_cast<int32_t*>(rec.data());
            int32_t* slot = hdr + 2;
            uint16_t* voff = reinterpret_cast<uint16_t*>(rec.data() + 40);
            uint16_t* ioff = reinterpret_cast<uint16_t*>(rec.data() + 56);
            uint16_t* len = reinterpret_cast<uint16_t*>(rec.data() + 72);
            double* invd = reinterpret_cast<double*>(rec.data() + 88);
            double* val = reinterpret_cast<double*>(rec.data() + val0);
            uint16_t* idx = reinterpret_cast<uint16_t*>(rec.data() + idx0);
            hdr[0] = is_long ? 1 : 0; hdr[1] = (int32_t)ne;
            size_t e = 0;
            for (int r = 0; r < 8; ++r) {
                slot[r] = -1; voff[r] = (uint16_t)(val0 / 8); ioff[r] = (uint16_t)(idx0 / 2); len[r] = 0; invd[r] = 0.0;
                const PkRow* row = is_long ? rs[0] : (r < nrows ? rs[r] : nullptr);
                if (!row) continue;
                if (is_long && r > 0) {
                    slot[r] = slot[0]; voff[r] = voff[0]; ioff[r] = ioff[0]; len[r] = len[0]; invd[r] = invd[0];
                    continue;
                }
                slot[r] = row->slot; invd[r] = row->invd; len[r] = (uint16_t)row->val.size();
                voff[r] = (uint16_t)((val0 + 8 * e) / 8); ioff[r] = (uint16_t)((idx0 + 2 * e) / 2);
                std::copy(row->val.begin(), row->val.end(), val + e);
                std::copy(row->idx.begin(), row->idx.end(), idx + e);
                e += row->val.size();
            }
            return rec;
        };
        for (int l = 0; l < new_depth; ++l) {
            std::vector<const PkRow*> longs, shorts;
            for (const PkRow& r : lv[l]) ((int)r.idx.size() > kLongRowNnz ? longs : shorts).push_back(&r);
            if (nr0 > kPkWarpRows && !shorts.empty()) {
                constexpr int kWarps = kPkThreads / 32;
                std::stable_sort(shorts.begin(), shorts.end(), [](const PkRow* a, const PkRow* b) { return a->idx.size() > b->idx.size(); });
                size_t promote = 0;
                while (promote < shorts.size() && shorts[promote]->idx.size() > 4 &&
                       longs.size() + promote + 1 + (shorts.size() - promote - 1 + 7) / 8 <= (size_t)kWarps) ++promote;
                longs.insert(longs.end(), shorts.begin(), shorts.begin() + promote);
                shorts.erase(shorts.begin(), shorts.begin() + promote);
            }
            std::stable_sort(longs.begin(), longs.end(), [](const PkRow* a, const PkRow* b) { return a->idx.size() > b->idx.size(); });
            bool first = true;
            for (const PkRow* r : longs) { add_record(make_record(&r, 1, true), first); first = false; }
            for (size_t q = 0; q < shorts.size(); q += 8) {
                add_record(make_record(shorts.data() + q, (int)std::min<size_t>(8, shorts.size() - q), false), first);
                first = false;
            }
        }
        close_chunk();
        for (int32_t u : C) cidx[u] = -1;
        if (nC == 0 && nr0 <= kPkWarpRows && P.bytes.size() <= (size_t)kPkChunk && P.last_used <= (size_t)kPkWarpBlob) {
            P.bytes.resize((P.last_used + 15) / 16 * 16);
            kind[t] = 1;
        } else {
            kind[t] = 2;
        }
    };
    if (H.n_sub > 0) {
        int nthreads = (int)std::min<int64_t>(std::max(1u, std::thread::hardware_concurrency()), 32);
        if (const char* e = getenv("CUADMM_INIT_THREADS")) nthreads = std::max(1, atoi(e));
        nthreads = (int)std::min<int64_t>(nthreads, H.n_sub);
        std::atomic<int64_t> next{0};
        std::vector<std::string> errors(nthreads);
        auto worker = [&](int id) {
            try {
                for (int64_t t = next.fetch_add(1); t < H.n_sub; t = next.fetch_add(1)) do_subtree(t);
            } catch (const std::exception& ex) { errors[id] = ex.what(); next.store(H.n_sub); }
        };
        std::vector<std::thread> pool;
        for (int i = 1; i < nthreads; ++i) pool.emplace_back(worker, i);
        worker(0);
        for (auto& th : pool) th.join();
        for (const std::string& e : errors) if (!e.empty()) throw Error(CUADMM_EINVAL, e);
        for (int64_t t = 0; t < H.n_sub; ++t) {
            if (kind[t] == 1) blobs.push_back(std::move(result[t]));
            else if (kind[t] == 2) packs.push_back(std::move(result[t]));
        }
    }
    n_collapsed = a_collapsed; levels_before = a_before; levels_after = a_after; chain_entries = a_entries;
    S.n_sub_pack = (int64_t)packs.size();
    S.n_sub_warp = (int64_t)blobs.size();
    S.pk_smem = 0; S.pk_rows = 0;
    if (packs.empty() && blobs.empty()) return;
    std::stable_sort(packs.begin(), packs.end(), [](const Packed& a, const Packed& b) { return a.bytes.size() > b.bytes.size(); });
    std::stable_sort(blobs.begin(), blobs.end(), [&](const Packed& a, const Packed& b) { return a.levels > b.levels; });
    std::vector<int64_t> chunk_off(1, 0), blob_off(1, 0), row_off(1, 0), ext_ptr(1, 0);
    std::vector<int32_t> prow_u, prow_src, prow_out, ext_dep;
    std::vector<double> ext_val;
    std::vector<unsigned char> stream, blob_bytes;
    int64_t max_slots = 0;
    auto add_slots = [&](const Packed& P) {
        for (size_t q = 0; q < P.slot_u.size(); ++q) {
            const int32_t u = P.slot_u[q], su = P.slot_src[q];
            prow_u.push_back(u);
            prow_out.push_back((u >= 0 && H.out_perm) ? (*H.out_perm)[u] : 0);
            prow_src.push_back(su < 0 ? -1 : (H.gather ? (*H.gather)[su] : su));
            if (su >= 0)
                for (int64_t p = H.ptr[su]; p < H.ptr[su + 1]; ++p)
                    if (!same(su, p)) { ext_dep.push_back(H.dep[p]); ext_val.push_back(H.val[p]); }
            ext_ptr.push_back((int64_t)ext_dep.size());
        }
        row_off.push_back((int64_t)prow_u.size());
        max_slots = std::max<int64_t>(max_slots, (int64_t)P.slot_u.size());
    };
    for (const Packed& P : packs) {
        stream.insert(stream.end(), P.bytes.begin(), P.bytes.end());
        stream.resize((stream.size() + kPkChunk - 1) / kPkChunk * kPkChunk, 0);
        chunk_off.push_back((int64_t)(stream.size() / kPkChunk));
        add_slots(P);
    }
    const int64_t cta_slots = max_slots;
    for (const Packed& P : blobs) {
        blob_bytes.insert(blob_bytes.end(), P.bytes.begin(), P.bytes.end());
        blob_off.push_back((int64_t)(blob_bytes.size() / 16));
        add_slots(P);
    }
    S.pk_rows = (int64_t)prow_u.size();
    S.pk_has_ext = !ext_dep.empty();
    if (ext_dep.empty()) { ext_dep.push_back(0); ext_val.push_back(0.0); }
    if (stream.empty()) stream.assign(16, 0);
    if (blob_bytes.empty()) blob_bytes.assign(16, 0);
    S.pk_stream.upload(stream); S.pk_chunk_off.upload(chunk_off); S.pk_blobs.upload(blob_bytes); S.pk_blob_off.upload(blob_off);
    S.pk_row_off.upload(row_off); S.pk_prow_u.upload(prow_u); S.pk_prow_src.upload(prow_src); S.pk_prow_out.upload(prow_out);
    S.pk_ext_ptr.upload(ext_ptr); S.pk_ext_dep.upload(ext_dep); S.pk_ext_val.upload(ext_val);
    S.pk_w.alloc(S.pk_rows);
    std::vector<int32_t> heavy;
    for (int64_t g = 0; g < S.pk_rows; ++g) if (ext_ptr[g + 1] - ext_ptr[g] > kPkHeavyExt) heavy.push_back((int32_t)g);
    S.pk_n_heavy = (int64_t)heavy.size();
    if (heavy.empty()) heavy.push_back(0);
    S.pk_heavy.upload(heavy);
    if (getenv("CUADMM_YSOLVE_TIMELINE") && !packs.empty()) {
        S.pk_timeline.alloc(4 * (int64_t)packs.size());
        std::vector<long long> meta;
        for (const Packed& P : packs) { meta.push_back((long long)((P.bytes.size() + kPkChunk - 1) / kPkChunk)); meta.push_back((long long)P.slot_u.size()); meta.push_back(P.levels); }
        S.pk_timeline_meta = meta;
    }
    S.pk_smem = (size_t)kPkRing * kPkChunk + 64 + sizeof(double) * (size_t)cta_slots;
    CUADMM_CUDA(cudaFuncSetAttribute((const void*)tri_packed_kernel, cudaFuncAttributeMaxDynamicSharedMemorySize, (int)S.pk_smem));
    if (verbose)
        fprintf(stderr, "[ysolve] %s packed: %zu CTA subtrees in %lld chunks (largest %zu), %zu warp subtrees in %zu bytes, "
                "%lld slots, %lld external entries (%lld heavy rows), smem %zu; chains collapsed in %lld subtrees (%lld -> %lld levels, %lld inverse entries)\n",
                H.subtrees_first ? "fwd" : "bwd", packs.size(), (long long)chunk_off.back(),
                packs.empty() ? (size_t)0 : (packs[0].bytes.size() + kPkChunk - 1) / kPkChunk, blobs.size(), blob_bytes.size(), (long long)S.pk_rows,
                (long long)ext_ptr.back(), (long long)S.pk_n_heavy, S.pk_smem, (long long)n_collapsed, (long long)levels_before, (long long)levels_after,
                (long long)chain_entries);
}

static void upload_sweep(const HostSweep& H, TriSweep& S) {
    S.n_unknowns = (int64_t)H.order.size();
    S.nnz = (int64_t)H.dep.size();
    S.subtrees_first = H.subtrees_first;
    std::vector<int32_t> level(H.n, 0);
    for (int32_t u : H.order) {
        int32_t l = 0;
        for (int64_t p = H.ptr[u]; p < H.ptr[u + 1]; ++p) {
            const int32_t d = H.dep[p];
            if (H.sub[d] == H.sub[u]) l = std::max(l, level[d] + 1);
        }
        level[u] = l;
    }
    std::vector<int32_t> slot_rows, slot_info;
    std::vector<std::vector<int32_t>> members(H.n_sub);
    std::vector<int32_t> depth(H.n_sub, 0);
    for (int32_t u : H.order) if (H.sub[u] >= 0) {
        members[H.sub[u]].push_back(u);
        depth[H.sub[u]] = std::max(depth[H.sub[u]], level[u] + 1);
    }
    std::vector<int> kind;
    pack_subtrees(H, S, members, level, depth, kind);
    std::vector<int32_t> sub_order;
    for (int64_t t = 0; t < H.n_sub; ++t) if (kind[t] == 0) sub_order.push_back((int32_t)t);
    std::stable_sort(sub_order.begin(), sub_order.end(), [&](int32_t a, int32_t b) { return depth[a] > depth[b]; });
    S.n_sub_cta = (int64_t)sub_order.size();
    std::vector<int64_t> sub_off(1, 0), sub_lvl_ptr;
    int max_sub_depth = 0;
    for (int32_t t : sub_order) {
        std::vector<std::vector<int32_t>> by_level(depth[t]);
        for (int32_t u : members[t]) by_level[level[u]].push_back(u);
        for (int l = 0; l < depth[t]; ++l) {
            sub_lvl_ptr.push_back((int64_t)slot_info.size());
            emit_level_slots(H, by_level[l], l, slot_rows, slot_info);
        }
        sub_lvl_ptr.push_back((int64_t)slot_info.size());
        sub_off.push_back((int64_t)sub_lvl_ptr.size());
    }
    for (int64_t t = 0; t < H.n_sub; ++t) max_sub_depth = std::max(max_sub_depth, depth[t]);
    S.n_sub = H.n_sub;
    S.sub_depth = max_sub_depth;
    if (getenv("CUADMM_YSOLVE_VERBOSE")) {
        const int64_t edges[] = {8, 32, 128, 256, 512, 1024, 2048, 4096, 1 << 30};
        for (int b = 0; b < 9; ++b) {
            int64_t cnt = 0, r = 0, dsum = 0; int dmax = 0;
            for (int64_t t = 0; t < H.n_sub; ++t) {
                const int64_t sz = (int64_t)members[t].size();
                if (sz <= edges[b] && (b == 0 || sz > edges[b - 1])) { ++cnt; r += sz; dsum += depth[t]; dmax = std::max(dmax, depth[t]); }
            }
            if (cnt) fprintf(stderr, "[ysolve]   rows<=%lld: %lld subtrees, %lld rows, sum depth %lld, max depth %d\n",
                             (long long)edges[b], (long long)cnt, (long long)r, (long long)dsum, dmax);
        }
    }
    int maxlev = -1;
    for (int32_t u : H.order) if (H.sub[u] < 0) maxlev = std::max(maxlev, (int)level[u]);
    S.levels = maxlev + 1;
    std::vector<std::vector<int32_t>> top_by_level(std::max(S.levels, 0));
    for (int32_t u : H.order) if (H.sub[u] < 0) top_by_level[level[u]].push_back(u);
    S.h_level_ptr.assign(S.levels + 1, (int64_t)slot_info.size());
    std::vector<int64_t> level_slots(std::max(S.levels, 1), 0);
    for (int l = 0; l < S.levels; ++l) {
        S.h_level_ptr[l] = (int64_t)slot_info.size();
        level_slots[l] = emit_level_slots(H, top_by_level[l], l, slot_rows, slot_info);
        S.h_level_ptr[l + 1] = (int64_t)slot_info.size();
    }
    S.n_slots = (int64_t)slot_info.size();
    int narrow_slots = kNarrowSlots;
    if (const char* e = getenv("CUADMM_SWEEP_NARROW_SLOTS")) narrow_slots = atoi(e);
    S.phases.clear();
    for (int l = 0; l < S.levels;) {
        if (level_slots[l] <= narrow_slots) {
            int e = l;
            while (e < S.levels && level_slots[e] <= narrow_slots) ++e;
            S.phases.push_back({true, l, e});
            l = e;
        } else {
            S.phases.push_back({false, l, l + 1});
            ++l;
        }
    }
    S.ptr.upload(H.ptr);
    std::vector<int32_t> dep(H.dep); if (dep.empty()) dep.push_back(0);
    std::vector<double> val(H.val); if (val.empty()) val.push_back(0.0);
    S.dep.upload(dep); S.val.upload(val);
    S.inv_diag.upload(H.inv_diag);
    if (slot_rows.empty()) { slot_rows.assign(8, -1); slot_info.push_back(0); }
    S.slot_rows.upload(slot_rows); S.slot_info.upload(slot_info);
    S.level_ptr.upload(S.h_level_ptr);
    if (sub_lvl_ptr.empty()) sub_lvl_ptr.push_back(0);
    S.sub_off.upload(sub_off); S.sub_lvl_ptr.upload(sub_lvl_ptr);
}

static int64_t choose_subtrees(const CholFactor& F, int64_t n_lead, std::vector<int32_t>& sub) {
    const int64_t n = F.n;
    sub.assign(n, -1);
    int64_t cap = 12000;
    if (const char* e = getenv("CUADMM_SWEEP_SUBTREE_CAP")) cap = atoll(e);
    if (cap <= 0) return 0;
    cap = std::min<int64_t>(cap, (int64_t)(232448 - kPkRing * kPkChunk - 64) / 8 - kPkChainMax);
    int64_t min_size = 2;
    if (const char* e = getenv("CUADMM_SWEEP_SUBTREE_MIN")) min_size = atoll(e);
    std::vector<int64_t> size(n, 1);
    for (int64_t v = 0; v < n_lead; ++v) {
        const int32_t p = F.parent[v];
        if (p >= 0 && p < n_lead) size[p] += size[v];
    }
    int64_t n_sub = 0;
    for (int64_t v = n_lead - 1; v >= 0; --v) {
        const int32_t p = F.parent[v];
        const bool parent_top = (p < 0 || p >= n_lead || sub[p] < 0);
        if (!parent_top) { sub[v] = sub[p]; continue; }
        const bool parent_fits = (p >= 0 && p < n_lead && size[p] <= cap);
        if (size[v] <= cap && !parent_fits && size[v] >= min_size) sub[v] = (int32_t)n_sub++;
    }
    return n_sub;
}

static int64_t choose_tail(const CholFactor& F, std::vector<int32_t>& level_out) {
    const int64_t n = F.n;
    std::vector<int32_t> lev(n, 0);
    for (int64_t j = 0; j < n; ++j)
        for (int64_t p = F.Lp[j] + 1; p < F.Lp[j + 1]; ++p) lev[F.Li[p]] = std::max(lev[F.Li[p]], lev[j] + 1);
    level_out = lev;
    int depth = 0;
    for (int64_t i = 0; i < n; ++i) depth = std::max(depth, lev[i] + 1);
    int64_t max_tail = 10240;
    int min_depth = 64;
    if (const char* e = getenv("CUADMM_YSOLVE_MAX_TAIL")) max_tail = atoll(e);
    if (const char* e = getenv("CUADMM_YSOLVE_MIN_DEPTH")) min_depth = atoi(e);
    if (depth <= min_depth || max_tail <= 0) return depth + 1;
    std::vector<int64_t> cnt(depth + 1, 0);
    for (int64_t i = 0; i < n; ++i) cnt[lev[i]]++;
    int64_t above = 0;
    int cut = depth;
    for (int l = depth - 1; l >= min_depth / 2; --l) {
        if (above + cnt[l] > max_tail) break;
        above += cnt[l];
        cut = l;
    }
    if (above < 32) return depth + 1;
    return cut;
}

cuadmm_ysolve_s* ysolve_create(int64_t m, int64_t vec_len, int64_t nnz, const int32_t* rowptr, const int32_t* colind,
                               const double* val, double eps, int device) {
    CUADMM_REQUIRE(m >= 0 && vec_len >= 0 && nnz >= 0, "negative dimension");
    CUADMM_REQUIRE(rowptr && (nnz == 0 || (colind && val)), "null argument");
    CUADMM_REQUIRE(rowptr[0] == 0 && rowptr[m] == nnz, "rowptr does not span nnz");
    int cnt = 0;
    if (cudaGetDeviceCount(&cnt) != cudaSuccess || cnt == 0) {
        cudaGetLastError();
        throw Error(CUADMM_ENODEVICE, "no CUDA device available; the y-solve has no CPU fallback");
    }
    CUADMM_REQUIRE(device >= 0 && device < cnt, "device index out of range");
    std::unique_ptr<cuadmm_ysolve_s> Y(new cuadmm_ysolve_s());
    Y->device = device; Y->m = m;
    DeviceGuard g(device);

    const bool vtime = getenv("CUADMM_YSOLVE_VERBOSE") != nullptr;
    auto tp0 = std::chrono::steady_clock::now();
    auto lap = [&](const char* what) {
        if (!vtime) return;
        const auto t = std::chrono::steady_clock::now();
        fprintf(stderr, "[ysolve] init %-28s %8.1f ms\n", what, std::chrono::duration<double, std::milli>(t - tp0).count());
        tp0 = t;
    };
    SymCsc M = form_aat(m, vec_len, rowptr, colind, val, eps);
    lap("A A^T");
    Y->nnz_aat = M.p[m];
    std::vector<int32_t> perm0 = min_degree_order(M);
    lap("minimum-degree ordering");
    CholFactor F;
    chol_symbolic(M, perm0, F, nullptr);
    lap("symbolic (1)");
    std::vector<int32_t> lev;
    const int64_t cut = choose_tail(F, lev);
    std::vector<int32_t> perm1; perm1.reserve(m);
    for (int64_t k = 0; k < m; ++k) if (lev[k] < cut) perm1.push_back(F.perm[k]);
    const int64_t n_lead = (int64_t)perm1.size();
    for (int64_t k = 0; k < m; ++k) if (lev[k] >= cut) perm1.push_back(F.perm[k]);
    const int64_t n_tail = m - n_lead;
    SymCsc C;
    if (n_tail > 0) {
        F = CholFactor();
        chol_symbolic(M, perm1, F, &C);
    } else {
        chol_symbolic(M, perm0, F, &C);
    }
    lap("symbolic (2, tail last)");
    chol_numeric(C, F, n_lead);
    lap("numeric (sparse lead part)");
    Y->n_lead = n_lead; Y->n_tail = n_tail;
    Y->nnz_L = F.nnz();
    Y->n_deficient = F.n_deficient;
    Y->h_perm = F.perm;
    Y->perm.upload(F.perm);

    std::vector<int32_t> sub;
    const int64_t n_sub = choose_subtrees(F, n_lead, sub);
    {
        HostSweep H;
        H.n = m;
        H.ptr.assign(m + 1, 0);
        for (int64_t j = 0; j < n_lead; ++j)
            for (int64_t p = F.Lp[j] + 1; p < F.Lp[j + 1]; ++p) H.ptr[F.Li[p] + 1]++;
        for (int64_t i = 0; i < m; ++i) H.ptr[i + 1] += H.ptr[i];
        H.dep.resize(H.ptr[m]); H.val.resize(H.ptr[m]);
        std::vector<int64_t> nx(H.ptr.begin(), H.ptr.end() - 1);
        for (int64_t j = 0; j < n_lead; ++j)
            for (int64_t p = F.Lp[j] + 1; p < F.Lp[j + 1]; ++p) {
                const int64_t q = nx[F.Li[p]]++;
                H.dep[q] = (int32_t)j; H.val[q] = F.Lx[p];
            }
        H.inv_diag.assign(m, 1.0);
        for (int64_t i = 0; i < n_lead; ++i) H.inv_diag[i] = 1.0 / F.Lx[F.Lp[i]];
        H.order.resize(m);
        std::iota(H.order.begin(), H.order.end(), 0);
        H.sub = sub; H.n_sub = n_sub; H.subtrees_first = true;
        H.gather = &Y->h_perm;
        upload_sweep(H, Y->fwd);
    }
    {
        HostSweep H;
        H.n = m;
        H.ptr.assign(m + 1, 0);
        for (int64_t j = 0; j < n_lead; ++j) H.ptr[j + 1] = F.Lp[j + 1] - F.Lp[j] - 1;
        for (int64_t i = 0; i < m; ++i) H.ptr[i + 1] += H.ptr[i];
        H.dep.resize(H.ptr[m]); H.val.resize(H.ptr[m]);
        for (int64_t j = 0; j < n_lead; ++j) {
            int64_t q = H.ptr[j];
            for (int64_t p = F.Lp[j] + 1; p < F.Lp[j + 1]; ++p, ++q) { H.dep[q] = F.Li[p]; H.val[q] = F.Lx[p]; }
        }
        H.inv_diag.assign(m, 1.0);
        for (int64_t i = 0; i < n_lead; ++i) H.inv_diag[i] = 1.0 / F.Lx[F.Lp[i]];
        H.order.resize(n_lead);
        for (int64_t j = 0; j < n_lead; ++j) H.order[j] = (int32_t)(n_lead - 1 - j);
        H.sub = sub;
        for (int64_t i = n_lead; i < m; ++i) H.sub[i] = -2;
        H.n_sub = n_sub; H.subtrees_first = false;
        H.out_perm = &Y->h_perm;
        upload_sweep(H, Y->bwd);
    }
    lap("pack + upload sweeps");
    Y->z.alloc(std::max<int64_t>(m, 1));
    Y->x.alloc(std::max<int64_t>(m, 1));

    if (n_tail > 0) {
        int64_t tail_def = 0;
        std::vector<int> flags;
        build_dense_tail(C, F, n_lead, n_tail, Y->tail_inv, Y->tail_inv_t, &tail_def, &flags);
        const int nt = (int)((n_tail + 63) / 64);
        std::vector<int32_t> tp(1, 0), tc, tpt(1, 0), tct;
        auto add_runs = [&](std::vector<int32_t>& ptr, std::vector<int32_t>& col, int J0, int J1, auto used) {
            for (int J = J0; J < J1;) {
                if (!used(J)) { ++J; continue; }
                int E = J;
                while (E < J1 && used(E)) ++E;
                col.push_back(J * 64); col.push_back(E * 64);
                J = E;
            }
            ptr.push_back((int32_t)(col.size() / 2));
        };
        Y->h_tail_cost[0].assign(nt, 0.0); Y->h_tail_cost[1].assign(nt, 0.0);
        for (int I = 0; I < nt; ++I) {
            add_runs(tp, tc, 0, I + 1, [&](int J) { return flags[(size_t)I * nt + J] != 0; });
            add_runs(tpt, tct, I, nt, [&](int J) { return flags[(size_t)J * nt + I] != 0; });
            for (int32_t t = tp[I]; t < tp[I + 1]; ++t) Y->h_tail_cost[0][I] += tc[2 * t + 1] - tc[2 * t];
            for (int32_t t = tpt[I]; t < tpt[I + 1]; ++t) Y->h_tail_cost[1][I] += tct[2 * t + 1] - tct[2 * t];
        }
        if (tc.empty()) tc.assign(2, 0);
        if (tct.empty()) tct.assign(2, 0);
        Y->tail_tptr.upload(tp); Y->tail_tcol.upload(tc); Y->tail_tptr_t.upload(tpt); Y->tail_tcol_t.upload(tct);
        Y->n_deficient += tail_def;
        Y->tail_tmp.alloc(n_tail);
        lap("dense tail (GPU)");
    }
    Y->launches_per_solve = (int)(Y->fwd.phases.size() + Y->bwd.phases.size()) + (n_tail > 0 ? 2 : 0) +
                            (Y->fwd.n_sub_cta > 0 ? 2 : 0) + (Y->fwd.n_sub_warp > 0 ? 2 : 0) + (Y->fwd.n_sub_pack > 0 ? 2 : 0) +
                            (Y->fwd.pk_rows > 0 ? 2 : 0);
    CUADMM_CUDA(cudaStreamCreateWithFlags(&Y->streams.side, cudaStreamNonBlocking));
    CUADMM_CUDA(cudaEventCreateWithFlags(&Y->streams.fork, cudaEventDisableTiming));
    CUADMM_CUDA(cudaEventCreateWithFlags(&Y->streams.join, cudaEventDisableTiming));
    Y->alg_bytes = 2 * (12 * Y->nnz_L + 8 * m) + 24 * m;
    CUADMM_CUDA(cudaDeviceSynchronize());
    return Y.release();
}

}

using namespace cuadmm;

cuadmm_ysolve_s::~cuadmm_ysolve_s() {
    if (streams.fork) cudaEventDestroy(streams.fork);
    if (streams.join) cudaEventDestroy(streams.join);
    if (streams.side) cudaStreamDestroy(streams.side);
}

void cuadmm_ysolve_s::enable_peer(const PeerComm* pc, size_t off_tmp, size_t off_x) {
    peer = pc;
    peer_tmp = pc->ptrs(off_tmp);
    peer_x = pc->ptrs(off_x);
    tail_tmp_p = pc->local<double>(off_tmp);
    x_p = pc->local<double>(off_x);
    if (n_tail > 0 && pc->world > 1) launches_per_solve += 1;
    split_tail_rows(pc->world, pc->rank);
}

void cuadmm_ysolve_s::split_tail_rows(int world, int rank) {
    for (int k = 0; k < 2; ++k) {
        const std::vector<double>& c = h_tail_cost[k];
        double total = 0.0;
        for (int64_t i = 0; i < n_tail; ++i) total += c[i >> 6] + 32.0;
        std::vector<int64_t> cut(world + 1, n_tail);
        cut[0] = 0;
        double acc = 0.0;
        int q = 1;
        for (int64_t i = 0; i < n_tail && q < world; ++i) {
            acc += c[i >> 6] + 32.0;
            while (q < world && acc >= total * q / world) cut[q++] = std::min<int64_t>(n_tail, (i + 1 + 7) / 8 * 8);
        }
        tail_row0[k] = cut[rank]; tail_row1[k] = cut[rank + 1];
    }
    const int64_t nrb = std::max<int64_t>(1, (std::max(tail_row1[0] - tail_row0[0], tail_row1[1] - tail_row0[1]) + 7) / 8);
    split_part.alloc(nrb * 8 * 8);
    split_count.alloc(nrb);
    split_count.zero();
    CUADMM_CUDA(cudaDeviceSynchronize());
}

void cuadmm_ysolve_s::solve(const double* d_rhs_, double* d_y_, cudaStream_t st) {
    if (m == 0) return;
    double* xv = x_p ? x_p : x.p;
    double* tmpv = tail_tmp_p ? tail_tmp_p : tail_tmp.p;
    launch_sweep(fwd, d_rhs_, perm.p, z.p, nullptr, nullptr, done_flag, st, streams);
    auto mark = [&](int tag) {
        if (!prof_ev) return;
        cudaEvent_t ev;
        CUADMM_CUDA(cudaEventCreate(&ev));
        CUADMM_CUDA(cudaEventRecord(ev, st));
        prof_ev->push_back(ev); prof_tag->push_back(tag);
    };
    auto gemv_split = [&](const double* Tm, const double* in, double* out, const int32_t* tp, const int32_t* tc, int longest_last,
                          int64_t r0, int64_t nrows_, int npush, const PeerView& pv, const PeerPtrs& outp) {
        const int64_t nrb = std::max<int64_t>(1, (nrows_ + 7) / 8);
        int splits = (int)std::min<int64_t>(8, std::max<int64_t>(1, (2 * 148 + nrb - 1) / nrb));
        CUADMM_REQUIRE(split_part.n >= nrb * 8 * 8 && split_count.n >= nrb, "internal: split-column GEMV scratch too small");
        tail_gemv_kernel<<<(unsigned)(nrb * splits), 256, 0, st>>>(n_tail, Tm, in, out, tp, tc, nullptr, nullptr, 0, done_flag,
            longest_last, r0, nrows_, npush, pv, outp, PeerPtrs(), splits, split_part.p, split_count.p);
    };
    if (n_tail > 0) {
        mark(20);
        if (!peer || peer->world == 1) {
            const int blocks = (int)((n_tail + 7) / 8);
            tail_gemv_row_kernel<<<blocks, 256, 0, st>>>(n_tail, tail_inv.p, z.p + n_lead, tmpv, tail_tptr.p, tail_tcol.p,
                                                         nullptr, nullptr, 0, done_flag, 1);
            tail_gemv_row_kernel<<<blocks, 256, 0, st>>>(n_tail, tail_inv_t.p, tmpv, xv + n_lead, tail_tptr_t.p, tail_tcol_t.p,
                                                         d_y_, perm.p, n_lead, done_flag, 0);
        } else {
            PeerPtrs pxt = peer_x;
            for (int q = 0; q < peer->world; ++q) pxt.p[q] += n_lead;
            const PeerView pv = peer->view();
            const int64_t n0 = tail_row1[0] - tail_row0[0], n1 = tail_row1[1] - tail_row0[1];
            gemv_split(tail_inv.p, z.p + n_lead, tmpv, tail_tptr.p, tail_tcol.p, 1, tail_row0[0], n0, peer->world, pv, peer_tmp);
            gemv_split(tail_inv_t.p, tmpv, xv + n_lead, tail_tptr_t.p, tail_tcol_t.p, 0, tail_row0[1], n1, peer->world, pv, pxt);
            tail_scatter_kernel<<<(int)((n_tail + 255) / 256), 256, 0, st>>>(n_tail, xv + n_lead, perm.p, n_lead, d_y_, done_flag);
        }
        CUADMM_CUDA(cudaGetLastError());
        mark(21);
    }
    launch_sweep(bwd, z.p, nullptr, xv, d_y_, perm.p, done_flag, st, streams);
}

extern "C" {

int cuadmm_ysolve_create(int64_t m, int64_t vec_len, int64_t nnz, const int32_t* h_A_rowptr, const int32_t* h_A_colind,
                         const double* h_A_val, double eps, int device, cuadmm_ysolve_t** out) {
    return guarded([&] {
        CUADMM_REQUIRE(out != nullptr, "out is null");
        *out = nullptr;
        *out = ysolve_create(m, vec_len, nnz, h_A_rowptr, h_A_colind, h_A_val, eps, device);
    });
}

void cuadmm_ysolve_destroy(cuadmm_ysolve_t* ys) { delete ys; }

int cuadmm_ysolve(cuadmm_ysolve_t* ys, const double* d_rhs, double* d_y, void* stream) {
    return guarded([&] {
        CUADMM_REQUIRE(ys && d_rhs && d_y, "null argument");
        DeviceGuard g(ys->device);
        ys->solve(d_rhs, d_y, (cudaStream_t)stream);
    });
}

int cuadmm_debug_ysolve_timeline(cuadmm_ysolve_t* ys, int which, long long* timeline, long long* meta, int64_t cap, int64_t* n) {
    return guarded([&] {
        CUADMM_REQUIRE(ys && n, "null argument");
        DeviceGuard g(ys->device);
        const cuadmm::TriSweep& S = which ? ys->bwd : ys->fwd;
        *n = S.pk_timeline.n / 4;
        if (!timeline || cap < *n || *n == 0) return;
        CUADMM_CUDA(cudaDeviceSynchronize());
        CUADMM_CUDA(cudaMemcpy(timeline, S.pk_timeline.p, sizeof(long long) * 4 * (size_t)*n, cudaMemcpyDeviceToHost));
        if (meta) std::copy(S.pk_timeline_meta.begin(), S.pk_timeline_meta.end(), meta);
    });
}

int cuadmm_ysolve_host(cuadmm_ysolve_t* ys, const double* h_rhs, double* h_y) {
    return guarded([&] {
        CUADMM_REQUIRE(ys && h_rhs && h_y, "null argument");
        DeviceGuard g(ys->device);
        if (ys->d_rhs.n != ys->m) { ys->d_rhs.alloc(std::max<int64_t>(ys->m, 1)); ys->d_y.alloc(std::max<int64_t>(ys->m, 1)); }
        ys->d_rhs.upload(h_rhs, ys->m);
        ys->solve(ys->d_rhs.p, ys->d_y.p, 0);
        ys->d_y.download(h_y, ys->m);
        CUADMM_CUDA(cudaStreamSynchronize(0));
    });
}

int cuadmm_ysolve_stats(const cuadmm_ysolve_t* ys, int64_t out[8]) {
    return guarded([&] {
        CUADMM_REQUIRE(ys && out, "null argument");
        out[0] = ys->nnz_aat; out[1] = ys->nnz_L; out[2] = std::max(ys->fwd.levels, ys->bwd.levels);
        out[3] = ys->n_tail; out[4] = ys->launches_per_solve; out[5] = ys->alg_bytes;
        out[6] = ys->n_deficient; out[7] = ys->fwd.n_sub * 100000 + ys->fwd.sub_depth;
    });
}

int cuadmm_ysolve_perm(const cuadmm_ysolve_t* ys, int32_t* perm) {
    return guarded([&] {
        CUADMM_REQUIRE(ys && perm, "null argument");
        std::copy(ys->h_perm.begin(), ys->h_perm.end(), perm);
    });
}

}
```

### cuadmm_b200/csrc/ysolve.h

```cpp
#pragma once
#include "common.h"
#include "chol_host.h"
#include "peer.h"

namespace cuadmm {

struct TriSweep {
    int64_t n_unknowns = 0;
    int64_t nnz = 0;
    DevBuf<int64_t> ptr;
    DevBuf<int32_t> dep;
    DevBuf<double> val;
    DevBuf<double> inv_diag;
    DevBuf<int32_t> slot_rows;
    DevBuf<int32_t> slot_info;
    DevBuf<int64_t> level_ptr;
    std::vector<int64_t> h_level_ptr;
    struct Phase { bool narrow; int level0, level1; };
    std::vector<Phase> phases;
    int64_t n_slots = 0;
    int levels = 0;
    DevBuf<int64_t> sub_off, sub_lvl_ptr;
    int64_t n_sub = 0;
    int64_t n_sub_cta = 0;
    int64_t n_sub_pack = 0, n_sub_warp = 0, pk_rows = 0;
    DevBuf<unsigned char> pk_stream, pk_blobs;
    DevBuf<int64_t> pk_chunk_off, pk_blob_off, pk_row_off, pk_ext_ptr;
    DevBuf<int32_t> pk_prow_u, pk_prow_src, pk_prow_out, pk_ext_dep, pk_heavy;
    int64_t pk_n_heavy = 0;
    DevBuf<double> pk_ext_val, pk_w;
    DevBuf<long long> pk_timeline;
    std::vector<long long> pk_timeline_meta;
    size_t pk_smem = 0;
    bool pk_has_ext = false;
    int sub_depth = 0;
    bool subtrees_first = true;
};

struct SweepStreams {
    cudaStream_t side = nullptr;
    cudaEvent_t fork = nullptr, join = nullptr;
};

}

struct cuadmm_ysolve_s {
    int device = -1;
    int64_t m = 0;
    int64_t n_lead = 0, n_tail = 0;
    int64_t nnz_aat = 0, nnz_L = 0, n_deficient = 0;
    cuadmm::TriSweep fwd, bwd;
    cuadmm::DevBuf<int32_t> perm;
    cuadmm::DevBuf<double> z;
    cuadmm::DevBuf<double> x;
    cuadmm::DevBuf<double> tail_inv, tail_inv_t, tail_tmp;
    cuadmm::DevBuf<int32_t> tail_tptr, tail_tcol, tail_tptr_t, tail_tcol_t;
    cuadmm::DevBuf<double> d_rhs, d_y;
    std::vector<int32_t> h_perm;
    const cuadmm::PeerComm* peer = nullptr;
    double* tail_tmp_p = nullptr;
    double* x_p = nullptr;
    cuadmm::PeerPtrs peer_tmp, peer_x;
    int64_t tail_row0[2] = {0, 0}, tail_row1[2] = {0, 0};
    std::vector<double> h_tail_cost[2];
    void enable_peer(const cuadmm::PeerComm* pc, size_t off_tmp, size_t off_x);
    void split_tail_rows(int world, int rank);
    cuadmm::DevBuf<double> split_part;
    cuadmm::DevBuf<unsigned int> split_count;
    const int* done_flag = nullptr;
    std::vector<cudaEvent_t>* prof_ev = nullptr;
    std::vector<int>* prof_tag = nullptr;
    cuadmm::SweepStreams streams;
    ~cuadmm_ysolve_s();
    int launches_per_solve = 0;
    int64_t alg_bytes = 0;
    void solve(const double* d_rhs, double* d_y, cudaStream_t stream);
};

namespace cuadmm {
cuadmm_ysolve_s* ysolve_create(int64_t m, int64_t vec_len, int64_t nnz, const int32_t* rowptr, const int32_t* colind,
                               const double* val, double eps, int device);
}
```

Measured before the change: 828.0.

## Reorder dense tail by elimination level and pack nonzero tiles of L22 inverse

Chooses the dense tail as the top elimination-tree levels and orders those rows last, then postorders the tail. The tail inverse is stored only as packed nonzero 64x64 tiles, one copy per direction, replacing the full dense inverse and its transpose. GEMV kernels read through tile offsets and a host-computed longest-first block order. This is meant to cut the bytes streamed per tail solve and improve load balance, at the cost of more setup complexity and indirection in the kernels.

```diff
diff --git a/cuadmm_b200/csrc/chol_host.cpp b/cuadmm_b200/csrc/chol_host.cpp
--- a/cuadmm_b200/csrc/chol_host.cpp
+++ b/cuadmm_b200/csrc/chol_host.cpp
@@ -266,16 +266,14 @@
     if (permuted) *permuted = std::move(C);
 }
 
-std::vector<int32_t> postorder_perm(const SymCsc& M, const std::vector<int32_t>& perm) {
-    CholFactor F;
-    chol_symbolic(M, perm, F, nullptr);
-    const int64_t n = F.n;
+static std::vector<int32_t> forest_postorder(const std::vector<int32_t>& parent) {
+    const int64_t n = (int64_t)parent.size();
     std::vector<int32_t> head(n, -1), nxt(n, -1);
-    for (int64_t j = n - 1; j >= 0; --j) if (F.parent[j] >= 0) { nxt[j] = head[F.parent[j]]; head[F.parent[j]] = (int32_t)j; }
+    for (int64_t j = n - 1; j >= 0; --j) if (parent[j] >= 0) { nxt[j] = head[parent[j]]; head[parent[j]] = (int32_t)j; }
     std::vector<int32_t> post; post.reserve(n);
     std::vector<int32_t> stack;
     for (int64_t r = 0; r < n; ++r) {
-        if (F.parent[r] >= 0) continue;
+        if (parent[r] >= 0) continue;
         stack.push_back((int32_t)r);
         while (!stack.empty()) {
             const int32_t v = stack.back();
@@ -284,9 +282,72 @@
             else { post.push_back(v); stack.pop_back(); }
         }
     }
-    std::vector<int32_t> out(n);
-    for (int64_t k = 0; k < n; ++k) out[k] = perm[post[k]];
+    return post;
+}
+
+std::vector<int32_t> postorder_perm(const SymCsc& M, const std::vector<int32_t>& perm) {
+    CholFactor F;
+    chol_symbolic(M, perm, F, nullptr);
+    const std::vector<int32_t> post = forest_postorder(F.parent);
+    std::vector<int32_t> out(F.n);
+    for (int64_t k = 0; k < F.n; ++k) out[k] = perm[post[k]];
     return out;
+}
+
+static int64_t choose_tail(const CholFactor& F, std::vector<int32_t>& level_out) {
+    const int64_t n = F.n;
+    std::vector<int32_t> lev(n, 0);
+    for (int64_t j = 0; j < n; ++j)
+        for (int64_t p = F.Lp[j] + 1; p < F.Lp[j + 1]; ++p) lev[F.Li[p]] = std::max(lev[F.Li[p]], lev[j] + 1);
+    level_out = lev;
+    int depth = 0;
+    for (int64_t i = 0; i < n; ++i) depth = std::max(depth, lev[i] + 1);
+    int64_t max_tail = 10240;
+    int min_depth = 64;
+    if (const char* e = getenv("CUADMM_YSOLVE_MAX_TAIL")) max_tail = atoll(e);
+    if (const char* e = getenv("CUADMM_YSOLVE_MIN_DEPTH")) min_depth = atoi(e);
+    if (depth <= min_depth || max_tail <= 0) return depth + 1;
+    std::vector<int64_t> cnt(depth + 1, 0);
+    for (int64_t i = 0; i < n; ++i) cnt[lev[i]]++;
+    int64_t above = 0;
+    int cut = depth;
+    for (int l = depth - 1; l >= min_depth / 2; --l) {
+        if (above + cnt[l] > max_tail) break;
+        above += cnt[l];
+        cut = l;
+    }
+    if (above < 32) return depth + 1;
+    return cut;
+}
+
+int64_t order_tail_last(const SymCsc& M, CholFactor& F, SymCsc& C) {
+    const int64_t m = M.n;
+    std::vector<int32_t> perm0 = min_degree_order(M);
+    F = CholFactor();
+    chol_symbolic(M, perm0, F, nullptr);
+    std::vector<int32_t> lev;
+    const int64_t cut = choose_tail(F, lev);
+    std::vector<int32_t> perm1; perm1.reserve(m);
+    for (int64_t k = 0; k < m; ++k) if (lev[k] < cut) perm1.push_back(F.perm[k]);
+    const int64_t n_lead = (int64_t)perm1.size();
+    for (int64_t k = 0; k < m; ++k) if (lev[k] >= cut) perm1.push_back(F.perm[k]);
+    if (n_lead < m) {
+        F = CholFactor();
+        chol_symbolic(M, perm1, F, &C);
+    } else {
+        chol_symbolic(M, perm0, F, &C);
+    }
+    return n_lead;
+}
+
+std::vector<int32_t> tail_postorder(const CholFactor& F, int64_t n_lead) {
+    const int64_t r = F.n - n_lead;
+    std::vector<int32_t> parent(r);
+    for (int64_t i = 0; i < r; ++i) parent[i] = F.parent[n_lead + i] >= 0 ? (int32_t)(F.parent[n_lead + i] - n_lead) : -1;
+    const std::vector<int32_t> post = forest_postorder(parent);
+    std::vector<int32_t> pos(r);
+    for (int64_t k = 0; k < r; ++k) pos[post[k]] = (int32_t)k;
+    return pos;
 }
 
 std::vector<int64_t> find_supernodes(const CholFactor& F, int64_t max_size) {
diff --git a/cuadmm_b200/csrc/chol_host.h b/cuadmm_b200/csrc/chol_host.h
--- a/cuadmm_b200/csrc/chol_host.h
+++ b/cuadmm_b200/csrc/chol_host.h
@@ -31,6 +31,10 @@
 std::vector<int64_t> find_supernodes(const CholFactor& F, int64_t max_size);
 
 void chol_symbolic(const SymCsc& M, const std::vector<int32_t>& perm, CholFactor& F, SymCsc* permuted = nullptr);
+
+int64_t order_tail_last(const SymCsc& M, CholFactor& F, SymCsc& C);
+
+std::vector<int32_t> tail_postorder(const CholFactor& F, int64_t n_lead);
 double pivot_tol();
 void chol_numeric(const SymCsc& Mperm, CholFactor& F, int64_t n_lead);
 
diff --git a/cuadmm_b200/csrc/debug_api.cpp b/cuadmm_b200/csrc/debug_api.cpp
--- a/cuadmm_b200/csrc/debug_api.cpp
+++ b/cuadmm_b200/csrc/debug_api.cpp
@@ -90,4 +90,18 @@
     });
 }
 
+int cuadmm_debug_tail_order(int64_t m, int64_t ncols, const int32_t* rowptr, const int32_t* colind, const double* val,
+                            double eps, int64_t* n_lead, int32_t* parent, int32_t* pos) {
+    return guarded([&] {
+        CUADMM_REQUIRE(rowptr && n_lead && parent && pos, "null argument");
+        SymCsc M = form_aat(m, ncols, rowptr, colind, val, eps);
+        CholFactor F; SymCsc C;
+        *n_lead = order_tail_last(M, F, C);
+        const int64_t r = m - *n_lead;
+        for (int64_t i = 0; i < r; ++i) parent[i] = F.parent[*n_lead + i] >= 0 ? (int32_t)(F.parent[*n_lead + i] - *n_lead) : -1;
+        const std::vector<int32_t> p = tail_postorder(F, *n_lead);
+        std::copy(p.begin(), p.end(), pos);
+    });
 }
+
+}
diff --git a/cuadmm_b200/csrc/dense.cu b/cuadmm_b200/csrc/dense.cu
--- a/cuadmm_b200/csrc/dense.cu
+++ b/cuadmm_b200/csrc/dense.cu
@@ -200,33 +200,55 @@
     if (symmetric && r[e] != c[e]) D[c[e] + (int64_t)r[e] * ld] = v[e];
 }
 
-__global__ void transpose_kernel(int64_t n, const double* __restrict__ in, double* __restrict__ out) {
-    __shared__ double tile[32][33];
-    const int64_t bx = (int64_t)blockIdx.x * 32, by = (int64_t)blockIdx.y * 32;
-    for (int j = threadIdx.y; j < 32; j += blockDim.y) {
-        const int64_t x = bx + threadIdx.x, y = by + j;
-        if (x < n && y < n) tile[j][threadIdx.x] = in[x + y * n];
-    }
-    __syncthreads();
-    for (int j = threadIdx.y; j < 32; j += blockDim.y) {
-        const int64_t x = by + threadIdx.x, y = bx + j;
-        if (x < n && y < n) out[x + y * n] = tile[threadIdx.x][j];
-    }
-}
-
-__global__ void tile_occupancy_kernel(int64_t r, int nt, const double* __restrict__ A, int* __restrict__ flags) {
+__global__ void tile_occupancy_kernel(int64_t r, int nt, const double* __restrict__ L, const int32_t* __restrict__ ipos,
+                                      int* __restrict__ flags) {
     const int I = blockIdx.y, J = blockIdx.x;
     int any = 0;
     for (int e = threadIdx.x; e < 64 * 64; e += blockDim.x) {
-        const int64_t i = (int64_t)I * 64 + e / 64, j = (int64_t)J * 64 + e % 64;
-        if (i < r && j < r && A[i * r + j] != 0.0) any = 1;
+        const int64_t i = (int64_t)I * 64 + e % 64, j = (int64_t)J * 64 + e / 64;
+        if (i < r && j < r && L[ipos[i] + (int64_t)ipos[j] * r] != 0.0) any = 1;
     }
     if (__syncthreads_or(any) && threadIdx.x == 0) flags[I * nt + J] = 1;
 }
 
-void build_dense_tail(const SymCsc& C, const CholFactor& F, int64_t n_lead, int64_t r,
-                      DevBuf<double>& tail_inv, DevBuf<double>& tail_inv_t, int64_t* n_deficient,
-                      std::vector<int>* tile_flags) {
+void tile_occupancy(int64_t r, const double* L, const int32_t* ipos, std::vector<int>& flags) {
+    cudaStream_t st = 0;
+    const int nt = (int)((r + 63) / 64);
+    DevBuf<int> d((int64_t)nt * nt);
+    d.zero(st);
+    tile_occupancy_kernel<<<dim3(nt, nt), 256, 0, st>>>(r, nt, L, ipos, d.p);
+    CUADMM_CUDA(cudaGetLastError());
+    flags.resize((size_t)nt * nt);
+    d.download(flags.data(), (int64_t)flags.size(), st);
+    CUADMM_CUDA(cudaStreamSynchronize(st));
+}
+
+__global__ void pack_tiles_kernel(int64_t r, const double* __restrict__ L, const int32_t* __restrict__ ipos, int transpose,
+                                  const int64_t* __restrict__ tiles, double* __restrict__ out) {
+    const int64_t* t = tiles + 4 * (int64_t)blockIdx.x;
+    const int64_t I = t[0], J = t[1], dst = t[2], w = t[3];
+    for (int e = threadIdx.x; e < 64 * 64; e += blockDim.x) {
+        const int i = e / 64, j = e % 64;
+        const int64_t a = I * 64 + i, b = J * 64 + j;
+        double v = 0.0;
+        if (a < r && b < r) v = transpose ? L[ipos[b] + (int64_t)ipos[a] * r] : L[ipos[a] + (int64_t)ipos[b] * r];
+        out[dst + i * w + j] = v;
+    }
+}
+
+void pack_tiles(int64_t r, const double* L, const int32_t* ipos, bool transpose, const std::vector<int64_t>& tiles, double* out) {
+    cudaStream_t st = 0;
+    const int64_t n = (int64_t)tiles.size() / 4;
+    if (n == 0) return;
+    DevBuf<int64_t> d;
+    d.upload(tiles, st);
+    pack_tiles_kernel<<<(unsigned)n, 256, 0, st>>>(r, L, ipos, transpose ? 1 : 0, d.p, out);
+    CUADMM_CUDA(cudaGetLastError());
+    CUADMM_CUDA(cudaStreamSynchronize(st));
+}
+
+void build_dense_tail(const SymCsc& C, const CholFactor& F, int64_t n_lead, int64_t r, DevBuf<double>& tail_inv,
+                      int64_t* n_deficient) {
     cudaStream_t st = 0;
     DevBuf<double> S(r * r);
     S.zero(st);
@@ -278,29 +300,8 @@
     info.download(&h_info, 1, st);
     CUADMM_CUDA(cudaStreamSynchronize(st));
     if (n_deficient) *n_deficient = h_info;
-    tail_inv_t.alloc(r * r);
-    trtri_lower(st, r, S.p, r, inv_diag.p, tail_inv_t.p, r);
     tail_inv.alloc(r * r);
-    dim3 grid((unsigned)((r + 31) / 32), (unsigned)((r + 31) / 32)), block(32, 8);
-    transpose_kernel<<<grid, block, 0, st>>>(r, tail_inv_t.p, tail_inv.p);
-    CUADMM_CUDA(cudaGetLastError());
-    CUADMM_CUDA(cudaStreamSynchronize(st));
-    {
-        const int nt = (int)((r + 63) / 64);
-        DevBuf<int> flags((int64_t)nt * nt);
-        flags.zero(st);
-        tile_occupancy_kernel<<<dim3(nt, nt), 256, 0, st>>>(r, nt, tail_inv.p, flags.p);
-        std::vector<int> h((size_t)nt * nt);
-        flags.download(h.data(), (int64_t)h.size(), st);
-        CUADMM_CUDA(cudaStreamSynchronize(st));
-        if (getenv("CUADMM_YSOLVE_VERBOSE")) {
-            int64_t lower = 0, used = 0;
-            for (int I = 0; I < nt; ++I) for (int J = 0; J <= I; ++J) { ++lower; used += h[(size_t)I * nt + J]; }
-            fprintf(stderr, "[ysolve] dense tail %lld: %lld of %lld lower 64x64 tiles of L22^-1 are non-zero (%.1f%%)\n",
-                    (long long)r, (long long)used, (long long)lower, 100.0 * (double)used / (double)lower);
-        }
-        if (tile_flags) tile_flags->swap(h);
-    }
-}
-
-}
+    trtri_lower(st, r, S.p, r, inv_diag.p, tail_inv.p, r);
+}
+
+}
diff --git a/cuadmm_b200/csrc/dense.h b/cuadmm_b200/csrc/dense.h
--- a/cuadmm_b200/csrc/dense.h
+++ b/cuadmm_b200/csrc/dense.h
@@ -11,8 +11,9 @@
                  const double* pivot_floor = nullptr);
 void trtri_lower(cudaStream_t st, int64_t n, const double* L, int64_t ldl, const double* inv_diag, double* Linv, int64_t ldi);
 
-void build_dense_tail(const SymCsc& Cperm, const CholFactor& F, int64_t n_lead, int64_t n_tail,
-                      DevBuf<double>& tail_inv, DevBuf<double>& tail_inv_t, int64_t* n_deficient = nullptr,
-                      std::vector<int>* tile_flags = nullptr);
+void build_dense_tail(const SymCsc& Cperm, const CholFactor& F, int64_t n_lead, int64_t n_tail, DevBuf<double>& tail_inv,
+                      int64_t* n_deficient = nullptr);
+void tile_occupancy(int64_t r, const double* L, const int32_t* ipos, std::vector<int>& flags);
+void pack_tiles(int64_t r, const double* L, const int32_t* ipos, bool transpose, const std::vector<int64_t>& tiles, double* out);
 
 }
diff --git a/cuadmm_b200/csrc/ysolve.cu b/cuadmm_b200/csrc/ysolve.cu
--- a/cuadmm_b200/csrc/ysolve.cu
+++ b/cuadmm_b200/csrc/ysolve.cu
@@ -373,36 +373,32 @@
 
 __global__ void __launch_bounds__(256) tail_gemv_row_kernel(int64_t r, const double* __restrict__ T, const double* __restrict__ in,
                                                         double* out, const int32_t* __restrict__ tile_ptr,
-                                                        const int32_t* __restrict__ tile_col, double* out_scatter,
+                                                        const int32_t* __restrict__ tile_col, const int64_t* __restrict__ tile_off,
+                                                        const int32_t* __restrict__ blk_order, double* out_scatter,
                                                         const int32_t* __restrict__ out_perm, int64_t perm_base,
-                                                        const int* __restrict__ done_flag, int longest_last) {
+                                                        const int* __restrict__ done_flag) {
     if (done_flag && *done_flag) return;
     const int lane = threadIdx.x & 31;
-    const int64_t cta = longest_last ? (int64_t)gridDim.x - 1 - blockIdx.x : blockIdx.x;
-    const int64_t row = cta * (blockDim.x >> 5) + (threadIdx.x >> 5);
+    const int64_t row = (int64_t)blk_order[blockIdx.x] * (blockDim.x >> 5) + (threadIdx.x >> 5);
     if (row >= r) return;
-    const double* Ti = T + row * r;
     const int I = (int)(row >> 6);
     double acc0 = 0.0, acc1 = 0.0;
-    const bool vec = (r & 1) == 0 && (reinterpret_cast<uintptr_t>(T) & 15) == 0;
     const bool in_al = (reinterpret_cast<uintptr_t>(in) & 15) == 0;
     for (int t = tile_ptr[I]; t < tile_ptr[I + 1]; ++t) {
         const int64_t j0 = tile_col[2 * t];
-        const int64_t j1 = min((int64_t)tile_col[2 * t + 1], r);
-        if (vec) {
-            const int64_t jv = j0 + ((j1 - j0) & ~(int64_t)1);
+        const int64_t w = tile_col[2 * t + 1] - j0;
+        const int64_t n = min(w, r - j0);
+        const int64_t nv = n & ~(int64_t)1;
+        const double* Ti = T + tile_off[t] + (row & 63) * w;
+        const double* x = in + j0;
 #pragma unroll 4
-            for (int64_t j = j0 + 2 * lane; j < jv; j += 64) {
-                const double2 a = __ldcs(reinterpret_cast<const double2*>(Ti + j));
-                const double2 b = in_al ? *reinterpret_cast<const double2*>(in + j) : make_double2(in[j], in[j + 1]);
-                acc0 = fma(a.x, b.x, acc0);
-                acc1 = fma(a.y, b.y, acc1);
-            }
-            if (lane == 0 && jv < j1) acc0 = fma(Ti[jv], in[jv], acc0);
-        } else {
-#pragma unroll 4
-            for (int64_t j = j0 + lane; j < j1; j += 32) acc0 = fma(Ti[j], in[j], acc0);
-        }
+        for (int64_t k = 2 * lane; k < nv; k += 64) {
+            const double2 a = __ldcs(reinterpret_cast<const double2*>(Ti + k));
+            const double2 b = in_al ? *reinterpret_cast<const double2*>(x + k) : make_double2(x[k], x[k + 1]);
+            acc0 = fma(a.x, b.x, acc0);
+            acc1 = fma(a.y, b.y, acc1);
+        }
+        if (lane == 0 && nv < n) acc0 = fma(Ti[nv], x[nv], acc0);
     }
     double acc = acc0 + acc1;
 #pragma unroll
@@ -415,9 +411,10 @@
 
 __global__ void __launch_bounds__(256) tail_gemv_kernel(int64_t r, const double* __restrict__ T, const double* in,
                                                         double* out, const int32_t* __restrict__ tile_ptr,
-                                                        const int32_t* __restrict__ tile_col, double* out_scatter,
+                                                        const int32_t* __restrict__ tile_col, const int64_t* __restrict__ tile_off,
+                                                        const int32_t* __restrict__ blk_order, double* out_scatter,
                                                         const int32_t* __restrict__ out_perm, int64_t perm_base,
-                                                        const int* __restrict__ done_flag, int longest_last,
+                                                        const int* __restrict__ done_flag,
                                                         int64_t row0, int64_t nrows, int npush, PeerView pv,
                                                         PeerPtrs outp, PeerPtrs scatp, int splits, double* split_part,
                                                         unsigned int* split_count) {
@@ -428,51 +425,52 @@
     unsigned long long ep = 0;
     if (npush) ep = peer_epoch(pv);
     const int sp = (int)(blockIdx.x % (unsigned)splits);
-    const int64_t rb = blockIdx.x / (unsigned)splits, nrb = gridDim.x / (unsigned)splits;
-    const int64_t cta = longest_last ? nrb - 1 - rb : rb;
-    const int64_t base = row0 + cta * 8;
+    const int64_t rb = blockIdx.x / (unsigned)splits;
+    const int64_t base = row0 + (int64_t)blk_order[rb] * 8;
     const int nr = (int)max((int64_t)0, min((int64_t)8, row0 + nrows - base));
     double acc[8];
 #pragma unroll
     for (int q = 0; q < 8; ++q) acc[q] = 0.0;
     if (nr > 0) {
         const int I = (int)(base >> 6);
-        const bool vec = (r & 1) == 0 && (reinterpret_cast<uintptr_t>(T) & 15) == 0 && (reinterpret_cast<uintptr_t>(in) & 15) == 0;
-        const double* Tb = T + base * r;
+        const bool vec = (reinterpret_cast<uintptr_t>(in) & 15) == 0;
         int g = 0;
         for (int t = tile_ptr[I]; t < tile_ptr[I + 1]; ++t) {
             const int64_t j0 = tile_col[2 * t];
-            const int64_t j1 = min((int64_t)tile_col[2 * t + 1], r);
-            const int nch = (int)((j1 - j0 + 63) >> 6);
+            const int64_t rw = tile_col[2 * t + 1] - j0;
+            const int64_t n = min(rw, r - j0);
+            const double* Tb = T + tile_off[t] + (base & 63) * rw;
+            const double* x = in + j0;
+            const int nch = (int)((n + 63) >> 6);
             const int g0 = g;
             int c = (w - (g & 7)) & 7;
             g += nch;
             for (; c < nch; c += 8) {
                 if (splits > 1 && (((g0 + c) >> 3) % splits) != sp) continue;
-                const int64_t j = j0 + ((int64_t)c << 6) + 2 * lane;
+                const int64_t k = ((int64_t)c << 6) + 2 * lane;
                 if (vec) {
-                    if (j + 1 < j1) {
-                        const double2 b = *reinterpret_cast<const double2*>(in + j);
+                    if (k + 1 < n) {
+                        const double2 b = *reinterpret_cast<const double2*>(x + k);
 #pragma unroll
                         for (int q = 0; q < 8; ++q) {
                             if (q < nr) {
-                                const double2 a = __ldcs(reinterpret_cast<const double2*>(Tb + q * r + j));
+                                const double2 a = __ldcs(reinterpret_cast<const double2*>(Tb + q * rw + k));
                                 acc[q] = fma(a.x, b.x, fma(a.y, b.y, acc[q]));
                             }
                         }
-                    } else if (j < j1) {
-                        const double b = in[j];
+                    } else if (k < n) {
+                        const double b = x[k];
 #pragma unroll
-                        for (int q = 0; q < 8; ++q) if (q < nr) acc[q] = fma(Tb[q * r + j], b, acc[q]);
+                        for (int q = 0; q < 8; ++q) if (q < nr) acc[q] = fma(Tb[q * rw + k], b, acc[q]);
                     }
                 } else {
 #pragma unroll
                     for (int h = 0; h < 2; ++h) {
-                        const int64_t jj = j0 + ((int64_t)c << 6) + lane + 32 * h;
-                        if (jj < j1) {
-                            const double b = in[jj];
+                        const int64_t kk = ((int64_t)c << 6) + lane + 32 * h;
+                        if (kk < n) {
+                            const double b = x[kk];
 #pragma unroll
-                            for (int q = 0; q < 8; ++q) if (q < nr) acc[q] = fma(Tb[q * r + jj], b, acc[q]);
+                            for (int q = 0; q < 8; ++q) if (q < nr) acc[q] = fma(Tb[q * rw + kk], b, acc[q]);
                         }
                     }
                 }
@@ -1049,30 +1047,88 @@
     return n_sub;
 }
 
-static int64_t choose_tail(const CholFactor& F, std::vector<int32_t>& level_out) {
-    const int64_t n = F.n;
-    std::vector<int32_t> lev(n, 0);
-    for (int64_t j = 0; j < n; ++j)
-        for (int64_t p = F.Lp[j] + 1; p < F.Lp[j + 1]; ++p) lev[F.Li[p]] = std::max(lev[F.Li[p]], lev[j] + 1);
-    level_out = lev;
-    int depth = 0;
-    for (int64_t i = 0; i < n; ++i) depth = std::max(depth, lev[i] + 1);
-    int64_t max_tail = 10240;
-    int min_depth = 64;
-    if (const char* e = getenv("CUADMM_YSOLVE_MAX_TAIL")) max_tail = atoll(e);
-    if (const char* e = getenv("CUADMM_YSOLVE_MIN_DEPTH")) min_depth = atoi(e);
-    if (depth <= min_depth || max_tail <= 0) return depth + 1;
-    std::vector<int64_t> cnt(depth + 1, 0);
-    for (int64_t i = 0; i < n; ++i) cnt[lev[i]]++;
-    int64_t above = 0;
-    int cut = depth;
-    for (int l = depth - 1; l >= min_depth / 2; --l) {
-        if (above + cnt[l] > max_tail) break;
-        above += cnt[l];
-        cut = l;
-    }
-    if (above < 32) return depth + 1;
-    return cut;
+static std::vector<int32_t> longest_first(const std::vector<double>& cost, int64_t row0, int64_t nrows) {
+    std::vector<int32_t> b((size_t)std::max<int64_t>(1, (nrows + 7) / 8));
+    std::iota(b.begin(), b.end(), 0);
+    if (nrows > 0)
+        std::stable_sort(b.begin(), b.end(), [&](int32_t x, int32_t y) { return cost[(row0 + 8 * x) >> 6] > cost[(row0 + 8 * y) >> 6]; });
+    return b;
+}
+
+static void pack_tail_matrix(int64_t r, const double* Linv, const int32_t* d_ipos, const std::vector<int>& flags, bool lower,
+                             TailMatrix& T) {
+    const int nt = (int)((r + 63) / 64);
+    std::vector<int32_t> ptr(1, 0), col;
+    std::vector<int64_t> off, tiles;
+    int64_t size = 0;
+    T.cost.assign(nt, 0.0);
+    for (int I = 0; I < nt; ++I) {
+        const int J0 = lower ? 0 : I, J1 = lower ? I + 1 : nt;
+        auto used = [&](int J) { return flags[lower ? (size_t)I * nt + J : (size_t)J * nt + I] != 0; };
+        for (int J = J0; J < J1;) {
+            if (!used(J)) { ++J; continue; }
+            int E = J;
+            while (E < J1 && used(E)) ++E;
+            const int64_t w = (int64_t)(E - J) * 64;
+            col.push_back(J * 64); col.push_back(E * 64);
+            off.push_back(size);
+            for (int K = J; K < E; ++K) { tiles.push_back(I); tiles.push_back(K); tiles.push_back(size + (K - J) * 64); tiles.push_back(w); }
+            size += 64 * w;
+            T.cost[I] += (double)w;
+            J = E;
+        }
+        ptr.push_back((int32_t)(col.size() / 2));
+    }
+    if (col.empty()) { col.assign(2, 0); off.push_back(0); }
+    T.val.alloc(std::max<int64_t>(size, 1));
+    pack_tiles(r, Linv, d_ipos, !lower, tiles, T.val.p);
+    T.tptr.upload(ptr); T.tcol.upload(col); T.toff.upload(off);
+    T.order.upload(longest_first(T.cost, 0, r));
+}
+
+static void build_tail(cuadmm_ysolve_s& Y, const SymCsc& C, const CholFactor& F, std::vector<int32_t>& pos, int64_t* n_def) {
+    const int64_t r = Y.n_tail;
+    const int nt = (int)((r + 63) / 64);
+    DevBuf<double> Linv;
+    build_dense_tail(C, F, Y.n_lead, r, Linv, n_def);
+    DevBuf<int32_t> d_ipos;
+    std::vector<int> flags;
+    auto scan = [&]() {
+        std::vector<int32_t> ipos(r);
+        for (int64_t i = 0; i < r; ++i) ipos[pos[i]] = (int32_t)i;
+        d_ipos.upload(ipos);
+        tile_occupancy(r, Linv.p, d_ipos.p, flags);
+    };
+    auto lower_used = [&]() {
+        int64_t used = 0;
+        for (int I = 0; I < nt; ++I) for (int J = 0; J <= I; ++J) used += flags[(size_t)I * nt + J];
+        return used;
+    };
+    const bool verbose = getenv("CUADMM_YSOLVE_VERBOSE") != nullptr;
+    int64_t used_before = -1;
+    if (verbose) {
+        const std::vector<int32_t> keep(pos);
+        std::iota(pos.begin(), pos.end(), 0);
+        scan();
+        used_before = lower_used();
+        pos = keep;
+    }
+    scan();
+    bool upper = false;
+    for (int I = 0; I < nt && !upper; ++I) for (int J = I + 1; J < nt; ++J) if (flags[(size_t)I * nt + J]) { upper = true; break; }
+    if (upper) {
+        std::iota(pos.begin(), pos.end(), 0);
+        scan();
+    }
+    if (verbose) {
+        const int64_t lower = (int64_t)nt * (nt + 1) / 2, used = lower_used();
+        fprintf(stderr, "[ysolve] dense tail %lld: non-zero lower 64x64 tiles of L22^-1: %lld of %lld (%.1f%%) in the tail order, "
+                "%lld (%.1f%%) stored%s\n", (long long)r, (long long)used_before, (long long)lower,
+                100.0 * (double)used_before / (double)lower, (long long)used, 100.0 * (double)used / (double)lower,
+                upper ? " (postorder left a tile above the diagonal: tail order kept)" : "");
+    }
+    pack_tail_matrix(r, Linv.p, d_ipos.p, flags, true, Y.tail[0]);
+    pack_tail_matrix(r, Linv.p, d_ipos.p, flags, false, Y.tail[1]);
 }
 
 cuadmm_ysolve_s* ysolve_create(int64_t m, int64_t vec_len, int64_t nnz, const int32_t* rowptr, const int32_t* colind,
@@ -1101,33 +1157,32 @@
     SymCsc M = form_aat(m, vec_len, rowptr, colind, val, eps);
     lap("A A^T");
     Y->nnz_aat = M.p[m];
-    std::vector<int32_t> perm0 = min_degree_order(M);
-    lap("minimum-degree ordering");
     CholFactor F;
-    chol_symbolic(M, perm0, F, nullptr);
-    lap("symbolic (1)");
-    std::vector<int32_t> lev;
-    const int64_t cut = choose_tail(F, lev);
-    std::vector<int32_t> perm1; perm1.reserve(m);
-    for (int64_t k = 0; k < m; ++k) if (lev[k] < cut) perm1.push_back(F.perm[k]);
-    const int64_t n_lead = (int64_t)perm1.size();
-    for (int64_t k = 0; k < m; ++k) if (lev[k] >= cut) perm1.push_back(F.perm[k]);
+    SymCsc C;
+    const int64_t n_lead = order_tail_last(M, F, C);
     const int64_t n_tail = m - n_lead;
-    SymCsc C;
-    if (n_tail > 0) {
-        F = CholFactor();
-        chol_symbolic(M, perm1, F, &C);
-    } else {
-        chol_symbolic(M, perm0, F, &C);
-    }
-    lap("symbolic (2, tail last)");
+    lap("ordering + symbolic (tail last)");
     chol_numeric(C, F, n_lead);
     lap("numeric (sparse lead part)");
     Y->n_lead = n_lead; Y->n_tail = n_tail;
     Y->nnz_L = F.nnz();
     Y->n_deficient = F.n_deficient;
-    Y->h_perm = F.perm;
-    Y->perm.upload(F.perm);
+
+    std::vector<int32_t> pos(n_tail);
+    std::iota(pos.begin(), pos.end(), 0);
+    if (n_tail > 0) {
+        const char* e = getenv("CUADMM_YSOLVE_TAIL_POSTORDER");
+        if (!(e && atoi(e) == 0)) pos = tail_postorder(F, n_lead);
+        int64_t tail_def = 0;
+        build_tail(*Y, C, F, pos, &tail_def);
+        Y->n_deficient += tail_def;
+        Y->tail_tmp.alloc(n_tail);
+        lap("dense tail (GPU)");
+    }
+    auto relabel = [&](int32_t u) { return u < n_lead ? u : (int32_t)(n_lead + pos[u - n_lead]); };
+    Y->h_perm.resize(m);
+    for (int64_t k = 0; k < m; ++k) Y->h_perm[relabel((int32_t)k)] = F.perm[k];
+    Y->perm.upload(Y->h_perm);
 
     std::vector<int32_t> sub;
     const int64_t n_sub = choose_subtrees(F, n_lead, sub);
@@ -1136,13 +1191,13 @@
         H.n = m;
         H.ptr.assign(m + 1, 0);
         for (int64_t j = 0; j < n_lead; ++j)
-            for (int64_t p = F.Lp[j] + 1; p < F.Lp[j + 1]; ++p) H.ptr[F.Li[p] + 1]++;
+            for (int64_t p = F.Lp[j] + 1; p < F.Lp[j + 1]; ++p) H.ptr[relabel(F.Li[p]) + 1]++;
         for (int64_t i = 0; i < m; ++i) H.ptr[i + 1] += H.ptr[i];
         H.dep.resize(H.ptr[m]); H.val.resize(H.ptr[m]);
         std::vector<int64_t> nx(H.ptr.begin(), H.ptr.end() - 1);
         for (int64_t j = 0; j < n_lead; ++j)
             for (int64_t p = F.Lp[j] + 1; p < F.Lp[j + 1]; ++p) {
-                const int64_t q = nx[F.Li[p]]++;
+                const int64_t q = nx[relabel(F.Li[p])]++;
                 H.dep[q] = (int32_t)j; H.val[q] = F.Lx[p];
             }
         H.inv_diag.assign(m, 1.0);
@@ -1162,7 +1217,7 @@
         H.dep.resize(H.ptr[m]); H.val.resize(H.ptr[m]);
         for (int64_t j = 0; j < n_lead; ++j) {
             int64_t q = H.ptr[j];
-            for (int64_t p = F.Lp[j] + 1; p < F.Lp[j + 1]; ++p, ++q) { H.dep[q] = F.Li[p]; H.val[q] = F.Lx[p]; }
+            for (int64_t p = F.Lp[j] + 1; p < F.Lp[j + 1]; ++p, ++q) { H.dep[q] = relabel(F.Li[p]); H.val[q] = F.Lx[p]; }
         }
         H.inv_diag.assign(m, 1.0);
         for (int64_t i = 0; i < n_lead; ++i) H.inv_diag[i] = 1.0 / F.Lx[F.Lp[i]];
@@ -1178,36 +1233,6 @@
     Y->z.alloc(std::max<int64_t>(m, 1));
     Y->x.alloc(std::max<int64_t>(m, 1));
 
-    if (n_tail > 0) {
-        int64_t tail_def = 0;
-        std::vector<int> flags;
-        build_dense_tail(C, F, n_lead, n_tail, Y->tail_inv, Y->tail_inv_t, &tail_def, &flags);
-        const int nt = (int)((n_tail + 63) / 64);
-        std::vector<int32_t> tp(1, 0), tc, tpt(1, 0), tct;
-        auto add_runs = [&](std::vector<int32_t>& ptr, std::vector<int32_t>& col, int J0, int J1, auto used) {
-            for (int J = J0; J < J1;) {
-                if (!used(J)) { ++J; continue; }
-                int E = J;
-                while (E < J1 && used(E)) ++E;
-                col.push_back(J * 64); col.push_back(E * 64);
-                J = E;
-            }
-            ptr.push_back((int32_t)(col.size() / 2));
-        };
-        Y->h_tail_cost[0].assign(nt, 0.0); Y->h_tail_cost[1].assign(nt, 0.0);
-        for (int I = 0; I < nt; ++I) {
-            add_runs(tp, tc, 0, I + 1, [&](int J) { return flags[(size_t)I * nt + J] != 0; });
-            add_runs(tpt, tct, I, nt, [&](int J) { return flags[(size_t)J * nt + I] != 0; });
-            for (int32_t t = tp[I]; t < tp[I + 1]; ++t) Y->h_tail_cost[0][I] += tc[2 * t + 1] - tc[2 * t];
-            for (int32_t t = tpt[I]; t < tpt[I + 1]; ++t) Y->h_tail_cost[1][I] += tct[2 * t + 1] - tct[2 * t];
-        }
-        if (tc.empty()) tc.assign(2, 0);
-        if (tct.empty()) tct.assign(2, 0);
-        Y->tail_tptr.upload(tp); Y->tail_tcol.upload(tc); Y->tail_tptr_t.upload(tpt); Y->tail_tcol_t.upload(tct);
-        Y->n_deficient += tail_def;
-        Y->tail_tmp.alloc(n_tail);
-        lap("dense tail (GPU)");
-    }
     Y->launches_per_solve = (int)(Y->fwd.phases.size() + Y->bwd.phases.size()) + (n_tail > 0 ? 2 : 0) +
                             (Y->fwd.n_sub_cta > 0 ? 2 : 0) + (Y->fwd.n_sub_warp > 0 ? 2 : 0) + (Y->fwd.n_sub_pack > 0 ? 2 : 0) +
                             (Y->fwd.pk_rows > 0 ? 2 : 0);
@@ -1241,7 +1266,7 @@
 
 void cuadmm_ysolve_s::split_tail_rows(int world, int rank) {
     for (int k = 0; k < 2; ++k) {
-        const std::vector<double>& c = h_tail_cost[k];
+        const std::vector<double>& c = tail[k].cost;
         double total = 0.0;
         for (int64_t i = 0; i < n_tail; ++i) total += c[i >> 6] + 32.0;
         std::vector<int64_t> cut(world + 1, n_tail);
@@ -1253,6 +1278,7 @@
             while (q < world && acc >= total * q / world) cut[q++] = std::min<int64_t>(n_tail, (i + 1 + 7) / 8 * 8);
         }
         tail_row0[k] = cut[rank]; tail_row1[k] = cut[rank + 1];
+        tail[k].rank_order.upload(longest_first(c, tail_row0[k], tail_row1[k] - tail_row0[k]));
     }
     const int64_t nrb = std::max<int64_t>(1, (std::max(tail_row1[0] - tail_row0[0], tail_row1[1] - tail_row0[1]) + 7) / 8);
     split_part.alloc(nrb * 8 * 8);
@@ -1273,29 +1299,31 @@
         CUADMM_CUDA(cudaEventRecord(ev, st));
         prof_ev->push_back(ev); prof_tag->push_back(tag);
     };
-    auto gemv_split = [&](const double* Tm, const double* in, double* out, const int32_t* tp, const int32_t* tc, int longest_last,
-                          int64_t r0, int64_t nrows_, int npush, const PeerView& pv, const PeerPtrs& outp) {
+    auto gemv_split = [&](const TailMatrix& T, const double* in, double* out, int64_t r0, int64_t nrows_, int npush,
+                          const PeerView& pv, const PeerPtrs& outp) {
         const int64_t nrb = std::max<int64_t>(1, (nrows_ + 7) / 8);
         int splits = (int)std::min<int64_t>(8, std::max<int64_t>(1, (2 * 148 + nrb - 1) / nrb));
-        CUADMM_REQUIRE(split_part.n >= nrb * 8 * 8 && split_count.n >= nrb, "internal: split-column GEMV scratch too small");
-        tail_gemv_kernel<<<(unsigned)(nrb * splits), 256, 0, st>>>(n_tail, Tm, in, out, tp, tc, nullptr, nullptr, 0, done_flag,
-            longest_last, r0, nrows_, npush, pv, outp, PeerPtrs(), splits, split_part.p, split_count.p);
+        CUADMM_REQUIRE(split_part.n >= nrb * 8 * 8 && split_count.n >= nrb && T.rank_order.n >= nrb,
+                       "internal: split-column GEMV scratch too small");
+        tail_gemv_kernel<<<(unsigned)(nrb * splits), 256, 0, st>>>(n_tail, T.val.p, in, out, T.tptr.p, T.tcol.p, T.toff.p,
+            T.rank_order.p, nullptr, nullptr, 0, done_flag, r0, nrows_, npush, pv, outp, PeerPtrs(), splits, split_part.p,
+            split_count.p);
     };
     if (n_tail > 0) {
         mark(20);
         if (!peer || peer->world == 1) {
             const int blocks = (int)((n_tail + 7) / 8);
-            tail_gemv_row_kernel<<<blocks, 256, 0, st>>>(n_tail, tail_inv.p, z.p + n_lead, tmpv, tail_tptr.p, tail_tcol.p,
-                                                         nullptr, nullptr, 0, done_flag, 1);
-            tail_gemv_row_kernel<<<blocks, 256, 0, st>>>(n_tail, tail_inv_t.p, tmpv, xv + n_lead, tail_tptr_t.p, tail_tcol_t.p,
-                                                         d_y_, perm.p, n_lead, done_flag, 0);
+            tail_gemv_row_kernel<<<blocks, 256, 0, st>>>(n_tail, tail[0].val.p, z.p + n_lead, tmpv, tail[0].tptr.p, tail[0].tcol.p,
+                                                         tail[0].toff.p, tail[0].order.p, nullptr, nullptr, 0, done_flag);
+            tail_gemv_row_kernel<<<blocks, 256, 0, st>>>(n_tail, tail[1].val.p, tmpv, xv + n_lead, tail[1].tptr.p, tail[1].tcol.p,
+                                                         tail[1].toff.p, tail[1].order.p, d_y_, perm.p, n_lead, done_flag);
         } else {
             PeerPtrs pxt = peer_x;
             for (int q = 0; q < peer->world; ++q) pxt.p[q] += n_lead;
             const PeerView pv = peer->view();
             const int64_t n0 = tail_row1[0] - tail_row0[0], n1 = tail_row1[1] - tail_row0[1];
-            gemv_split(tail_inv.p, z.p + n_lead, tmpv, tail_tptr.p, tail_tcol.p, 1, tail_row0[0], n0, peer->world, pv, peer_tmp);
-            gemv_split(tail_inv_t.p, tmpv, xv + n_lead, tail_tptr_t.p, tail_tcol_t.p, 0, tail_row0[1], n1, peer->world, pv, pxt);
+            gemv_split(tail[0], z.p + n_lead, tmpv, tail_row0[0], n0, peer->world, pv, peer_tmp);
+            gemv_split(tail[1], tmpv, xv + n_lead, tail_row0[1], n1, peer->world, pv, pxt);
             tail_scatter_kernel<<<(int)((n_tail + 255) / 256), 256, 0, st>>>(n_tail, xv + n_lead, perm.p, n_lead, d_y_, done_flag);
         }
         CUADMM_CUDA(cudaGetLastError());
diff --git a/cuadmm_b200/csrc/ysolve.h b/cuadmm_b200/csrc/ysolve.h
--- a/cuadmm_b200/csrc/ysolve.h
+++ b/cuadmm_b200/csrc/ysolve.h
@@ -42,6 +42,15 @@
     cudaEvent_t fork = nullptr, join = nullptr;
 };
 
+struct TailMatrix {
+    DevBuf<double> val;
+    DevBuf<int32_t> tptr, tcol;
+    DevBuf<int64_t> toff;
+    DevBuf<int32_t> order;
+    DevBuf<int32_t> rank_order;
+    std::vector<double> cost;
+};
+
 }
 
 struct cuadmm_ysolve_s {
@@ -53,8 +62,8 @@
     cuadmm::DevBuf<int32_t> perm;
     cuadmm::DevBuf<double> z;
     cuadmm::DevBuf<double> x;
-    cuadmm::DevBuf<double> tail_inv, tail_inv_t, tail_tmp;
-    cuadmm::DevBuf<int32_t> tail_tptr, tail_tcol, tail_tptr_t, tail_tcol_t;
+    cuadmm::TailMatrix tail[2];
+    cuadmm::DevBuf<double> tail_tmp;
     cuadmm::DevBuf<double> d_rhs, d_y;
     std::vector<int32_t> h_perm;
     const cuadmm::PeerComm* peer = nullptr;
@@ -62,7 +71,6 @@
     double* x_p = nullptr;
     cuadmm::PeerPtrs peer_tmp, peer_x;
     int64_t tail_row0[2] = {0, 0}, tail_row1[2] = {0, 0};
-    std::vector<double> h_tail_cost[2];
     void enable_peer(const cuadmm::PeerComm* pc, size_t off_tmp, size_t off_x);
     void split_tail_rows(int world, int rank);
     cuadmm::DevBuf<double> split_part;
```

After: 949.3 (median of 6 runs). +14.6%, better.
